# MichaelMillerCSU/Koopman-online-updated-MPC

Hardware: AMD Instinct MI355X
Metric: MPC steps/s (lift+EDMD-update+QP, N=20, 20-dim lift) (higher is better)
Workload: dtype f64

## Files before the change

include/koopmpc.h:

```cpp
#ifndef KOOPMPC_H
#define KOOPMPC_H

#include <stdint.h>

#ifdef __cplusplus
extern "C" {
#endif

typedef struct kmpc_handle kmpc_handle;

enum { KMPC_F32 = 0, KMPC_F64 = 1 };
enum {
  KMPC_LIFT_MLP = 0,
  KMPC_LIFT_RBF_PY = 1,
  KMPC_LIFT_RBF_MATLAB = 2,
  KMPC_LIFT_RBF_GAUSS = 3,
  KMPC_LIFT_RBF_INVQUAD = 4,
  KMPC_LIFT_RBF_INVMULTQUAD = 5,
  KMPC_LIFT_RBF_POLYHARMONIC = 6
};
enum {
  KMPC_OUT_CX = 0,
  KMPC_OUT_LIFT = 1
};
// ... 36 lines not shown
const char* kmpc_last_error(const kmpc_handle* h);
int kmpc_version(void);

int kmpc_set_encoder(kmpc_handle* h, int layer, const double* W_host, const double* b_host,
                     int rows, int cols);
int kmpc_set_encoder_layer(kmpc_handle* h, int layer, const double* W_host, const double* b_host,
                           int rows, int cols);
int kmpc_set_centres(kmpc_handle* h, const double* cx_host, int L, int n);
int kmpc_set_rbf_order(kmpc_handle* h, int k);
int kmpc_set_model(kmpc_handle* h, const double* A_host, const double* B_host, const double* C_host);

int kmpc_set_terminal_weight(kmpc_handle* h, const double* PN);
int kmpc_reset(kmpc_handle* h, void* stream);
int kmpc_state_init(kmpc_handle* h, double P0_scale, double barQ0_scale, void* stream);
int kmpc_state_init_from(kmpc_handle* h, const double* K_A0, const double* P0, const double* barX0,
                         const double* barQ0, void* stream);

int kmpc_lift(kmpc_handle* h, const void* X_dev, void* Psi_dev, int B, void* stream);

int kmpc_rls_update(kmpc_handle* h, const void* psi_dev, const void* u_dev, const void* psi_next_dev,
                    const void* x_next_dev, int B, void* stream);

int kmpc_get_model(kmpc_handle* h, void* A_dev, void* B_dev, void* C_dev, void* stream);

int kmpc_condense(kmpc_handle* h, const void* psi_dev, const void* ref_dev, int ref_per_traj,
                  void* H_dev, void* f_dev, int B, void* stream);
int kmpc_condense_cost(kmpc_handle* h, const void* psi_dev, const void* ref_dev, int ref_per_traj,
                       void* H_dev, void* f_dev, void* c_dev, int B, void* stream);

int kmpc_mpc_solve(kmpc_handle* h, const void* A_dev, const void* B_dev, const void* C_dev, int model_shared,
                   const void* psi_dev, const void* ref_dev, int ref_per_traj, double lb, double ub, double Qw,
                   double Rw, const double* PN_host, void* U_dev, void* U0_dev, void* fun_dev, int32_t* status_dev,
                   int32_t* iters_dev, int B, void* stream);

int kmpc_qp_solve(kmpc_handle* h, const void* H_dev, const void* f_dev, void* U_dev,
                  int32_t* status_dev, int32_t* iters_dev, int B, void* stream);

int kmpc_step(kmpc_handle* h, const void* X_dev, const void* ref_dev, int ref_per_traj,
              void* U0_dev, void* Useq_dev, int32_t* status_dev, int32_t* iters_dev, void* stream);

int64_t kmpc_gram_elems(const kmpc_handle* h);
int kmpc_allreduce_gram(kmpc_handle* h, double* delta_gram_dev, void* nccl_comm, void* stream);
int kmpc_shared_local_gram(kmpc_handle* h, const void* X_dev, double* delta_gram_dev, void* stream);
int kmpc_gram_accumulate(kmpc_handle* h, const void* X_dev, double* delta_gram_dev, void* stream);
int kmpc_shared_solve(kmpc_handle* h, const double* delta_gram_dev, const void* ref_dev, void* U0_dev,
                      void* Useq_dev, int32_t* status_dev, int32_t* iters_dev, void* stream);
int kmpc_shared_solve_plant(kmpc_handle* h, const double* delta_gram_dev, const void* ref_dev, void* U0_dev, void* Useq_dev,
                            int32_t* status_dev, int32_t* iters_dev, int plant, void* X_dev, int switched, double hstep,
                            void* stream);
int kmpc_shared_rollout(kmpc_handle* h, int plant, void* X_dev, const void* ref_dev, int steps, int step0, int switch_step, double hstep,
                        void* nccl_comm, void* U_log_dev, void* X_log_dev, void* U0_dev, void* Useq_dev, int32_t* status_dev,
                        int32_t* iters_dev, void* stream);
int kmpc_shared_get_model(kmpc_handle* h, void* A_dev, void* B_dev, void* C_dev, void* stream);

int kmpc_offline_fit(kmpc_handle* h, const void* X_dev, const void* Y_dev, const void* U_dev, int M,
                     double ridge, int init_rls, void* A_dev, void* B_dev, void* C_dev, void* stream);
int kmpc_generate_and_fit(kmpc_handle* h, int plant, const void* X0_dev, const void* U_dev, int n_traj, int n_steps,
                          double hstep, double ridge, int init_rls, void* A_dev, void* B_dev, void* C_dev,
                          void* X_out_dev, void* Y_out_dev, void* stream);

int kmpc_set_applied_input(kmpc_handle* h, const void* U_dev, int B, void* stream);

int kmpc_plant_step(kmpc_handle* h, int plant, void* X_dev, const void* U_dev, double hstep,
                    int switched, int B, void* stream);

int kmpc_rollout(kmpc_handle* h, int plant, void* X_dev, const void* ref_dev, int ref_per_traj,
                 int steps, int step0, int switch_step, double hstep, void* U_log_dev, void* X_log_dev,
                 int32_t* status_dev, int32_t* iters_dev, void* stream);

int kmpc_solve_dare(const void* A, const void* B, const double* Q, double R, int maxiter, double eps, int nb,
                    int L, void* P, void* K, int32_t* iters, void* stream);
int kmpc_terminal_from_dare(kmpc_handle* h, const double* Q, double R, int maxiter, double eps,
                            int per_trajectory, double* PN_out, int32_t* iters_out, void* stream);

int kmpc_set_terminal_refresh(kmpc_handle* h, int every, const double* Q_host, double R, int maxiter, double eps);

int64_t kmpc_state_bytes(const kmpc_handle* h);
int kmpc_state_export(kmpc_handle* h, void* host_blob, int64_t bytes);
int kmpc_state_import(kmpc_handle* h, const void* host_blob, int64_t bytes);

int kmpc_profile_enable(kmpc_handle* h, int on);
int kmpc_profile_read(kmpc_handle* h, double* ms2, int64_t* count, int reset);
int kmpc_rollout_is_fused(const kmpc_handle* h);
int kmpc_rollout_plugin_status(const kmpc_handle* h, char* text, int text_bytes);
int kmpc_rollout_plugin_prebuild(int n, int L, int N, int out_rows, int lift_kind, int hidden_eff, int batch, int dtype, char* text,
                                 int text_bytes);
int kmpc_rank_by_work(const int32_t* work_dev, int B, int32_t* perm_dev, void* stream);
int kmpc_set_rollout_workgroup(int trajectories);
int64_t kmpc_algorithmic_bytes_per_step(const kmpc_handle* h);
int kmpc_set_online_update(kmpc_handle* h, int on);

int kmpc_set_rollout_diagnostics(kmpc_handle* h, int on);
int kmpc_rollout_diag(kmpc_handle* h, int plant, void* X_dev, const void* ref_dev, int ref_per_traj, int steps, int step0,
                      int switch_step, double hstep, void* U_log_dev, void* X_log_dev, void* Psi_log_dev, void* dA_log_dev,
                      void* dB_log_dev, void* dC_log_dev, int32_t* status_dev, int32_t* iters_dev, void* stream);
int kmpc_estimator_status(const kmpc_handle* h, double* P0, double* barQ0);
int kmpc_get_prev_transition(kmpc_handle* h, void* psi_prev_dev, void* u_prev_dev, void* stream);
int kmpc_rollout_diag_plugin_prebuild(int n, int L, int N, int out_rows, int lift_kind, int hidden_eff, int batch, int with_term,
                                      char* text, int text_bytes);

#ifdef __cplusplus
}
#endif
#endif
```

koopman-online-updated-mpc_amd/csrc/api.hip:

```cpp
#include <hip/hip_runtime.h>

#include <cmath>
#include <cstdio>
#include <cstring>
#include <string>
#include <vector>

#include "../../include/koopmpc.h"
#include "kernels.h"
#include <dlfcn.h>
#include <rccl/rccl.h>

using namespace kmpc;

static thread_local std::string g_create_error;

struct kmpc_handle {
  kmpc_config cfg{};
  std::string err;
  virtual ~kmpc_handle() {
    for (auto& mk : marks) (void)hipEventDestroy(mk.e);
  }
  virtual int set_encoder_layer(int layer, const double* W, const double* b, int rows, int cols) = 0;
  virtual int set_centres(const double* cx, int L, int n) = 0;
  virtual int set_rbf_order(int k) = 0;
  virtual int set_model(const double* A, const double* B, const double* C) = 0;
  virtual int set_terminal_weight(const double* PN) = 0;
  virtual int terminal_from_dare(const double* Qh, double R, int maxiter, double eps, int per_traj, double* PN_out,
                                 int32_t* iters_out, hipStream_t s) = 0;
  virtual int set_terminal_refresh(int every, const double* Qh, double R, int maxiter, double eps) = 0;
  virtual int rollout_is_fused() const = 0;
  virtual int rollout_plugin_status(std::string* text) const = 0;
  virtual int reset(hipStream_t s) = 0;
  virtual int state_init(double P0, double barQ0, hipStream_t s) = 0;
  virtual int state_init_from(const double* KA0, const double* P0m, const double* barX0, const double* barQ0m, hipStream_t s) = 0;
  virtual int lift(const void* X, void* Psi, int B, hipStream_t s) = 0;
  virtual int rls_update(const void* psi, const void* u, const void* psin, const void* xn, int B, hipStream_t s) = 0;
  virtual int get_model(void* A, void* B, void* C, hipStream_t s) = 0;
  virtual int condense(const void* psi, const void* ref, int rpt, void* H, void* f, void* c, int B, hipStream_t s) = 0;
  virtual int mpc_solve(const void* A, const void* Bv, const void* C, int shared, const void* psi, const void* ref, int rpt,
                        double lb, double ub, double Qw, double Rw, const double* PN, void* U, void* U0, void* fun,
                        int32_t* st, int32_t* it, int B, hipStream_t s) = 0;
  virtual int generate_and_fit(int plant, const void* X0, const void* U, int n_traj, int n_steps, double hs, double ridge,
                               int init_rls, void* A, void* B, void* C, void* Xo, void* Yo, hipStream_t s) = 0;
  int device = 0;
  struct StreamMark { hipStream_t s; hipEvent_t e; unsigned long long age; };
  std::vector<StreamMark> marks;
  unsigned long long mark_clock = 0;
  void mark_stream(hipStream_t s) {
    hipStreamCaptureStatus cap = hipStreamCaptureStatusNone;
    if (hipStreamIsCapturing(s, &cap) != hipSuccess) { (void)hipGetLastError(); return; }
    if (cap != hipStreamCaptureStatusNone) return;
    StreamMark* m = nullptr;
    for (auto& mk : marks)
      if (mk.s == s) { m = &mk; break; }
    if (!m) {
      if (marks.size() >= 16) {
        m = &marks[0];
        for (auto& mk : marks)
          if (mk.age < m->age) m = &mk;
        (void)hipEventSynchronize(m->e);
        m->s = s;
      } else {
        hipEvent_t e = nullptr;
        if (hipEventCreateWithFlags(&e, hipEventDisableTiming) != hipSuccess) { (void)hipGetLastError(); return; }
        marks.push_back(StreamMark{s, e, 0});
        m = &marks.back();
      }
    }
    m->age = ++mark_clock;
    if (hipEventRecord(m->e, s) != hipSuccess) (void)hipGetLastError();
  }
  hipError_t sync_marks() {
    for (auto& mk : marks) {
      const hipError_t e = hipEventSynchronize(mk.e);
      if (e != hipSuccess) return e;
    }
    return hipSuccess;
  }
  virtual int qp_solve(const void* H, const void* f, void* U, int32_t* st, int32_t* it, int B, hipStream_t s) = 0;
  virtual int step(const void* X, const void* ref, int rpt, void* U0, void* Useq, int32_t* st, int32_t* it,
                   hipStream_t s) = 0;
  virtual int plant_step(int plant, void* X, const void* U, double h, int sw, int B, hipStream_t s) = 0;
  virtual int set_applied_input(const void* U, int B, hipStream_t s) = 0;
  virtual int set_online_update(int on) = 0;
  virtual int rollout(int plant, void* X, const void* ref, int rpt, int steps, int step0, int switch_step, double hs,
                      void* Ulog, void* Xlog, int32_t* st, int32_t* it, hipStream_t s) = 0;
  virtual int set_rollout_diagnostics(int on) = 0;
  virtual int estimator_status(double* P0, double* barQ0) const = 0;
  virtual int get_prev_transition(void* psi_prev, void* u_prev, hipStream_t s) = 0;
  virtual int rollout_diag(int plant, void* X, const void* ref, int rpt, int steps, int step0, int switch_step, double hs, void* Ulog,
                           void* Xlog, void* Psilog, void* dAlog, void* dBlog, void* dClog, int32_t* st, int32_t* it, hipStream_t s) = 0;
  virtual int offline_fit(const void* X, const void* Y, const void* U, int M, double ridge, int init_rls, void* A,
                          void* B, void* C, hipStream_t s) = 0;
  virtual int64_t gram_elems() const = 0;
  virtual int shared_local_gram(const void* X, double* delta, hipStream_t s) = 0;
  virtual int shared_solve_plant(const double* delta, const void* ref, void* U0, void* Useq, int32_t* st, int32_t* it, int plant, void* X,
                                 int switched, double hstep, hipStream_t s) = 0;
  virtual int shared_solve(const double* delta, const void* ref, void* U0, void* Useq, int32_t* st, int32_t* it,
                           hipStream_t s) = 0;
  virtual int shared_get_model(void* A, void* B, void* C, hipStream_t s) = 0;
  virtual int shared_rollout(int plant, void* X, const void* ref, int steps, int step0, int switch_step, double hstep, void* comm,
                             void* Ulog, void* Xlog, void* U0out, void* Useq, int32_t* st, int32_t* it, hipStream_t s) = 0;
  virtual int64_t state_bytes() const = 0;
  virtual int state_export(void* blob, int64_t bytes) = 0;
  virtual int state_import(const void* blob, int64_t bytes) = 0;
  virtual int profile_enable(int on) = 0;
  virtual int profile_read(double* ms2, int64_t* count, int reset) = 0;
  virtual int64_t algorithmic_bytes() const = 0;
};

static void* resolve_nccl_allreduce() {
  static void* fn = nullptr;
  if (!fn) {
// ... 997 lines not shown
      if ((rc = pack_encoder(s))) return rc;
      r.lift_rbf = 0;
      r.W1 = dW1; r.b1 = db1; r.Whp[0] = dWhp[0]; r.Whp[1] = dWhp[1]; r.bh[0] = dbh[0]; r.bh[1] = dbh[1];
      r.Wop = dWop; r.bo = dbo; r.Hp = enc.Hp; r.Lp = enc.Lp; r.KS = enc.KS; r.nhh = cfg.layers - 1;
    } else {
      r.lift_rbf = 1;
      r.cx = dcx; r.eps = (T)cfg.rbf_eps; r.rbf_matlab = rbf_code();
    }
    r.psi[0] = dPsi[0]; r.psi[1] = dPsi[1]; r.cur = cur;
    r.steps = steps; r.step0 = step0; r.switch_step = switch_step;
    r.have_prev = have_prev ? 1 : 0; r.rls_fresh = rls_fresh ? 1 : 0;
    r.no_update = update_on ? 0 : 1;
    r.U_log = (T*)Ulog; r.X_log = (T*)Xlog;
    r.io_f32 = io32 ? 1 : 0;
    if (io32 && !r.s.U0) r.s.U0 = dU0;
    if (ctx.diag) { r.diag = 1; r.Psi_log = (T*)ctx.diag->Psi; r.dA_log = (T*)ctx.diag->dA; r.dB_log = (T*)ctx.diag->dB; r.dC_log = (T*)ctx.diag->dC; }
    if constexpr (sizeof(T) == 8) {
      if (term_every > 0) {
        if (io32) FAIL(-3, "the per-step terminal refresh is a float64 feature");
        r.term_every = term_every; r.term_count0 = (int)(term_count % term_every); r.term_maxiter = term_maxiter;
        r.term_R = term_R; r.term_eps = term_eps; r.term_Q = dTermQ; r.term_W = dWtB;
        r.term_scratch = dTermScr; r.term_scratch_stride = term_scratch_elems(L); r.term_iters = dDareIt;
        r.s.Wterm = dWtB; r.s.wterm_per_traj = 1;
      }
    }
    const bool global_place = cfg.lift_kind == KMPC_LIFT_MLP && (B & 15) == 0 && B <= (1 << 20);
    if (!dbg_env("KMPC_ROLLOUT_NO_PLACE")) {
      if (!dWork) {
        HIPCHK(hipMalloc(&dWork, sizeof(int32_t) * (size_t)B));
        HIPCHK(hipMemsetAsync(dWork, 0, sizeof(int32_t) * (size_t)B, s));
      }
      r.work = dWork;
      static const int tail = dbg_env("KMPC_PLACE_TAIL") ? atoi(dbg_env("KMPC_PLACE_TAIL")) : 5;
      r.work_tail = tail;
      if (place_valid && global_place && !dbg_env("KMPC_ROLLOUT_NO_GLOBAL_PLACE")) r.perm = dPerm;
      if (evPlace && place_stream != s) HIPCHK(hipStreamWaitEvent(s, evPlace, 0));
    }
    if constexpr (sizeof(T) == 8) {
      if (use_img) {
        if ((rc = ensure_image(s))) return rc;
        r.img = dImg; r.img_stride = sImg;
      } else if ((rc = ensure_dense(s, true))) return rc;
    }
    bool rec;
    if ((rc = prof_begin(s, &rec)) || (rec && (rc = prof_mid(s)))) return rc;
    HIPCHK(launch_rollout_fused<T>(r, s, &variant_of(ctx.diag != nullptr).plugin));
    if (rec && (rc = prof_end(s, steps))) return rc;
    if (r.work && steps >= 4 && global_place) {
      if (!dPerm) HIPCHK(hipMalloc(&dPerm, sizeof(int32_t) * (size_t)B * 3));
      HIPCHK(launch_place(dWork, B, dPerm, reinterpret_cast<uint32_t*>(dPerm + B), s));
      place_valid = true;
    } else {
      place_valid = false;
    }
    if (r.work) {
      if (!evPlace) HIPCHK(hipEventCreateWithFlags(&evPlace, hipEventDisableTiming));
      HIPCHK(hipEventRecord(evPlace, s));
      place_stream = s;
    }
    if (term_every > 0) term_count += steps;
    if (update_on && (steps >= 2 || (steps == 1 && have_prev))) rls_fresh = false;
    have_prev = true;
    cur ^= (steps & 1);
    return 0;
  }

  T* dU0 = nullptr;
  int rollout(int plant, void* X, const void* ref, int rpt, int steps, int step0, int switch_step, double hs,
              void* Ulog, void* Xlog, int32_t* st, int32_t* it, hipStream_t s) override {
    return rollout_impl(StepCtx{}, plant, X, ref, rpt, steps, step0, switch_step, hs, Ulog, Xlog, st, it, s);
  }
  int rollout_impl(const StepCtx& ctx, int plant, void* X, const void* ref, int rpt, int steps, int step0, int switch_step, double hs,
                   void* Ulog, void* Xlog, int32_t* st, int32_t* it, hipStream_t s) {
    if (!X || !ref || steps < 0) FAIL(-3, "kmpc_rollout: bad arguments");
    if (!dU0) HIPCHK(hipMalloc(&dU0, sizeof(T) * (size_t)B));
    if (n != 2) FAIL(-3, "plants are two-state systems");
    if (!plant_id_ok(plant)) FAIL(-3, "unknown plant");
    const bool fused = fused_rollout_ok() && (!ctx.diag || diag_fused_ready());
    const bool kernel_writes_totals = steps > 0 && fused && cfg.lift_kind == KMPC_LIFT_MLP;
    if (!kernel_writes_totals) {
      if (st) HIPCHK(hipMemsetAsync(st, 0, sizeof(int32_t) * (size_t)B, s));
      if (it) HIPCHK(hipMemsetAsync(it, 0, sizeof(int32_t) * (size_t)B, s));
    }
    if (steps > 0 && fused)
      return rollout_fused(ctx, plant, X, ref, rpt, steps, step0, switch_step, hs, Ulog, Xlog, st, it, s);
    if (steps == 0 && fused) {
      if constexpr (sizeof(T) == 8) {
        if (use_img) return ensure_image(s);
      } else if (core) {
        int rc = ensure_image(s);
        if (!rc && core->use_img && (rc = core->ensure_image(s))) err = core->err;
        return rc;
      }
      return 0;
    }
    for (int i = 0; i < steps; ++i) {
      const int gi = step0 + i;
      T* u = Ulog ? (T*)Ulog + (size_t)i * B : dU0;
      if (ctx.diag) { const int rcd = diag_before_step(*ctx.diag, X, i, s); if (rcd) return rcd; }
      int rc = step_impl(StepCtx{true, plant, (switch_step >= 0 && gi >= switch_step) ? 1 : 0, hs, X, nullptr}, X, ref, rpt, u, nullptr, st, it, s);
      if (rc) return rc;
      if (Xlog) HIPCHK(hipMemcpyAsync((T*)Xlog + (size_t)i * n * B, X, sizeof(T) * (size_t)n * B,
                                      hipMemcpyDeviceToDevice, s));
    }
    return 0;
  }

  double *dGram = nullptr, *dPartial = nullptr;
  T *dKs = nullptr, *dCs = nullptr, *dHs = nullptr, *dFs = nullptr, *df0s = nullptr, *dTs = nullptr;
  double* dFastPack = nullptr;
  bool fast_pack_valid = false;
  int32_t* dNeed = nullptr;
  int32_t* dWork = nullptr;
  int32_t* dPerm = nullptr;
  bool place_valid = false;
  hipEvent_t evPlace = nullptr;
  hipStream_t place_stream = nullptr;
  int32_t* dQpList = nullptr;
  int qp_list_parity = 0;
  T* dWt = nullptr;
  std::vector<double> hostPN;
  bool have_wterm = false;
  double* dDareP = nullptr; int32_t* dDareIt = nullptr; double* dWtB = nullptr;
  int dare_cap = 0;
  bool wterm_from_dare = false, wterm_per_traj = false;
  bool shared_has_samples = false;
  static constexpr int GRAM_BLOCKS = 256;
  int64_t gram_elems() const override { return (int64_t)(p + L + n) * p; }
  int shared_alloc() {
    if (dGram) return 0;
    const int R = p + L + n, MT = (R + 15) / 16, NT = (p + 15) / 16;
    HIPCHK(hipMalloc(&dGram, sizeof(double) * (size_t)R * p));
    HIPCHK(hipMemset(dGram, 0, sizeof(double) * (size_t)R * p));
    HIPCHK(hipMalloc(&dPartial, sizeof(double) * (size_t)GRAM_BLOCKS * MT * 16 * NT * 16));
    HIPCHK(hipMalloc(&dKs, sizeof(T) * (size_t)L * p));
    HIPCHK(hipMalloc(&dCs, sizeof(T) * (size_t)n * L));
    HIPCHK(hipMalloc(&dHs, sizeof(T) * (size_t)N * N));
    HIPCHK(hipMalloc(&dFs, sizeof(T) * (size_t)N * (L + 1)));
    HIPCHK(hipMalloc(&df0s, sizeof(T) * (size_t)N));
    { int rc = sync_own(); if (rc) return rc; }
    { int rc = ensure_dense(nullptr, false); if (rc) return rc; HIPCHK(hipStreamSynchronize(nullptr)); }
    HIPCHK(hipMemcpy(dKs, dK, sizeof(T) * (size_t)L * p, hipMemcpyDeviceToDevice));
    HIPCHK(hipMemcpy(dCs, dC, sizeof(T) * (size_t)n * L, hipMemcpyDeviceToDevice));
    return 0;
  }
  int shared_local_gram(const void* X, double* delta, hipStream_t s) override {
    if (!X || !delta) FAIL(-3, "kmpc_shared_local_gram: null pointer");
    int rc = shared_alloc();
    if (rc) return rc;
    if (core && (rc = ensure_dense(s, true))) return rc;
    T* psi_now = dPsi[cur];
    T* psi_prev = dPsi[cur ^ 1];
    GramArgs<T> g{};
    g.B = B; g.n = n; g.L = L; g.max_blocks = GRAM_BLOCKS;
    g.psi_prev = psi_prev; g.pp_sl = 1; g.pp_sb = L;
    g.psi_now = psi_now; g.pn_sl = 1; g.pn_sb = L;
    g.u_prev = dUprev; g.x_now = (const T*)X; g.partial = dPartial;
    if constexpr (sizeof(T) == 8) {
      const bool two = dbg_env("KMPC_SHARED_LIFT_GRAM_2") != nullptr;
      if (have_prev && !two && cfg.lift_kind == KMPC_LIFT_MLP) {
        if ((rc = check_lift_ready())) return rc;
        LiftArgs<T> a{};
        a.B = B; a.n = n; a.L = L; a.hidden = enc.hid; a.nlayers = cfg.layers;
        a.X = (const T*)X; a.Psi = psi_now; a.ps_l = 1; a.ps_b = L;
        a.W1 = dW1; a.b1 = db1; a.Wh[0] = dWh[0]; a.Wh[1] = dWh[1]; a.bh[0] = dbh[0]; a.bh[1] = dbh[1];
        a.Wo = dWo; a.bo = dbo; a.Hp = enc.Hp; a.Lp = enc.Lp;
        if ((rc = pack_encoder(s))) return rc;
        a.Whp[0] = dWhp[0]; a.Whp[1] = dWhp[1] ? dWhp[1] : dWhp[0]; a.Wop = dWop; a.KSp = enc.KS;
// ... 351 lines not shown
    return 0;
  }

  int64_t algorithmic_bytes() const override {
    const int64_t s = sizeof(T);
    return s * (2 * ((int64_t)p * p + L * p + L * L + n * L) + (L + L * p + n * L + N * m + n) + (n + m + q * N));
  }
};

struct DeviceGuard {
  int prev = -1;
  explicit DeviceGuard(int dev) { if (hipGetDevice(&prev) != hipSuccess) prev = -1; if (prev != dev) (void)hipSetDevice(dev); else prev = -1; }
  ~DeviceGuard() { if (prev >= 0) (void)hipSetDevice(prev); }
};
extern "C" {

int kmpc_version(void) { return 100; }

int kmpc_create(const kmpc_config* cfg, kmpc_handle** out) {
  if (!cfg || !out) { g_create_error = "kmpc_create: null argument"; return -1; }
  *out = nullptr;
  int ndev = 0;
  if (hipGetDeviceCount(&ndev) != hipSuccess || ndev == 0) {
    g_create_error = "kmpc_create: no HIP device visible (libkoopmpc has no CPU path)";
    return -5;
  }
  kmpc_handle* h = nullptr;
  int rc;
  if (cfg->dtype == KMPC_F64) { auto* i = new Impl<double>(); rc = i->init(*cfg); h = i; }
  else if (cfg->dtype == KMPC_F32) { auto* i = new Impl<float>(); rc = i->init(*cfg); h = i; }
  else { g_create_error = "kmpc_create: dtype must be KMPC_F32 or KMPC_F64"; return -2; }
  if (rc) { g_create_error = h->err; delete h; return rc; }
  if (hipGetDevice(&h->device) != hipSuccess) h->device = 0;
  *out = h;
  return 0;
}

int kmpc_destroy(kmpc_handle* h) {
  if (!h) return 0;
  DeviceGuard g(h->device);
  delete h;
  return 0;
}
const char* kmpc_last_error(const kmpc_handle* h) { return h ? h->err.c_str() : g_create_error.c_str(); }

#define NN(h) if (!(h)) return -1; DeviceGuard dev_guard_((h)->device)
struct StreamMarkAtExit {
  kmpc_handle* h; hipStream_t s;
  ~StreamMarkAtExit() { h->mark_stream(s); }
};
#define NNS(h, s) NN(h); StreamMarkAtExit mark_at_exit_{(h), (hipStream_t)(s)}
int kmpc_set_encoder(kmpc_handle* h, int layer, const double* W, const double* b, int rows, int cols) { NN(h); return h->set_encoder_layer(layer, W, b, rows, cols); }
int kmpc_set_encoder_layer(kmpc_handle* h, int layer, const double* W, const double* b, int rows, int cols) { return kmpc_set_encoder(h, layer, W, b, rows, cols); }
int kmpc_set_centres(kmpc_handle* h, const double* cx, int L, int n) { NN(h); return h->set_centres(cx, L, n); }
int kmpc_set_rbf_order(kmpc_handle* h, int k) { NN(h); return h->set_rbf_order(k); }
int kmpc_set_model(kmpc_handle* h, const double* A, const double* B, const double* C) { NN(h); return h->set_model(A, B, C); }
int kmpc_set_terminal_weight(kmpc_handle* h, const double* PN) { NN(h); return h->set_terminal_weight(PN); }
int kmpc_terminal_from_dare(kmpc_handle* h, const double* Q, double R, int maxiter, double eps, int per_trajectory,
                            double* PN_out, int32_t* iters_out, void* s) {
  NNS(h, s);
  return h->terminal_from_dare(Q, R, maxiter, eps, per_trajectory, PN_out, iters_out, (hipStream_t)s);
}
int kmpc_solve_dare(const void* A, const void* B, const double* Q, double R, int maxiter, double eps, int nb, int L,
                    void* P, void* K, int32_t* iters, void* s) {
  if (nb == 0) return 0;
  if (!A || !B || !Q || !P || nb < 0 || L < 1 || L > 64 || maxiter < 1) return -3;
  double* dQl = nullptr;
  if (hipMalloc(&dQl, sizeof(double) * (size_t)L * L) != hipSuccess) return -1001;
  int rc = 0;
  if (hipMemcpyAsync(dQl, Q, sizeof(double) * (size_t)L * L, hipMemcpyHostToDevice, (hipStream_t)s) != hipSuccess) rc = -1002;
  DareArgs d{};
  d.nb = nb; d.L = L; d.q = 0; d.maxiter = maxiter; d.shared_model = 0;
  d.A = (const double*)A; d.strideA = (long)L * L; d.ldA = L;
  d.B = (const double*)B; d.strideB = L; d.incB = 1;
  d.Q = dQl; d.R = R; d.eps = eps; d.Co = nullptr; d.strideC = 0;
  d.P = (double*)P; d.K = (double*)K; d.PN = nullptr; d.pn_sub_diag = 0.0; d.iters = iters;
  if (!rc && launch_dare(d, (hipStream_t)s) != hipSuccess) rc = -1003;
  if (hipStreamSynchronize((hipStream_t)s) != hipSuccess && !rc) rc = -1004;
  (void)hipFree(dQl);
  return rc;
}
int kmpc_set_terminal_refresh(kmpc_handle* h, int every, const double* Q, double R, int maxiter, double eps) { NN(h); return h->set_terminal_refresh(every, Q, R, maxiter, eps); }
int kmpc_rollout_is_fused(const kmpc_handle* h) { NN(h); return h->rollout_is_fused(); }
static void put_text(char* text, int text_bytes, const std::string& t) { if (text && text_bytes > 0) snprintf(text, (size_t)text_bytes, "%s", t.c_str()); }
static int prebuild_variant(int n, int L, int N, int q, bool rbf, int hidden_eff, int batch, bool io32, bool term, bool diag, std::string* text, bool rbf_kinds) {
  const EncoderShape e = encoder_shape(hidden_eff, 0, n, L);
  RolloutPluginKey k{};
  if (!rollout_plugin_key(n, L, N, q, rbf, e.Lp, e.KS, e.Hp, batch, io32, &k, term, diag, rbf_kinds)) return 0;
  if (!rollout_plugin_get(k, text)) return -1;
  *text = rollout_plugin_describe(k);
  return 1;
}
int kmpc_rollout_plugin_prebuild(int n, int L, int N, int out_rows, int lift_kind, int hidden_eff, int batch, int dtype, char* text, int text_bytes) {
  auto say = [&](int code, const std::string& t) { put_text(text, text_bytes, t); return code; };
  const bool rbf = lift_kind != KMPC_LIFT_MLP, io32 = dtype == KMPC_F32;
  const int q = out_rows > 0 ? out_rows : n;
  if (lift_kind < KMPC_LIFT_MLP || lift_kind > KMPC_LIFT_RBF_POLYHARMONIC) return say(-3, "lift_kind must be one of KMPC_LIFT_* (0..6)");
  if (n != 2 || L < 1 || N < 1 || batch < 1 || (!rbf && (hidden_eff < 1 || hidden_eff > 128)) || (dtype != KMPC_F32 && dtype != KMPC_F64)) return say(-3, "bad arguments");
  if (!(io32 ? rollout_io32_available(n, L, N, q, rbf) : rollout_fused_available<double>(n, L, N, q, 64, rbf))) return say(2, "no fused roll-out for this configuration");
  std::string t;
  const int rc = prebuild_variant(n, L, N, q, rbf, hidden_eff, batch, io32, false, false, &t, lift_kind >= KMPC_LIFT_RBF_GAUSS);
  return rc == 0 ? say(0, "built-in instantiation of libkoopmpc.so") : say(rc, t);
}
int kmpc_rollout_diag_plugin_prebuild(int n, int L, int N, int out_rows, int lift_kind, int hidden_eff, int batch, int with_term, char* text, int text_bytes) {
  auto say = [&](int code, const std::string& t) { put_text(text, text_bytes, t); return code; };
  const bool rbf = lift_kind != KMPC_LIFT_MLP;
  const int q = out_rows > 0 ? out_rows : n;
  if (lift_kind < KMPC_LIFT_MLP || lift_kind > KMPC_LIFT_RBF_POLYHARMONIC) return say(-3, "lift_kind must be one of KMPC_LIFT_* (0..6)");
  if (n != 2 || L < 1 || N < 1 || batch < 1 || (!rbf && (hidden_eff < 1 || hidden_eff > 128))) return say(-3, "bad arguments");
  std::string t;
  const int rc = rollout_fused_available<double>(n, L, N, q, 64, rbf) ? prebuild_variant(n, L, N, q, rbf, hidden_eff, batch, false, with_term != 0, true, &t, lift_kind >= KMPC_LIFT_RBF_GAUSS) : 0;
  return rc == 0 ? say(2, "no fused diagnostics variant for this configuration (per-step launches)") : say(rc, t);
}
int kmpc_rollout_plugin_status(const kmpc_handle* h, char* text, int text_bytes) {
  if (!h) return -100;
  std::string t;
  const int rc = h->rollout_plugin_status(&t);
  put_text(text, text_bytes, t);
  return rc;
}
int kmpc_rank_by_work(const int32_t* work_dev, int B, int32_t* perm_dev, void* s) {
  if (!work_dev || !perm_dev) return -3;
  const hipError_t e = kmpc::launch_place(work_dev, B, perm_dev, reinterpret_cast<uint32_t*>(perm_dev + B), (hipStream_t)s);
  return e == hipSuccess ? 0 : -(1000 + (int)e);
}
int kmpc_set_rollout_workgroup(int trajectories) {
  if (trajectories != 0 && trajectories != 4 && trajectories != 8 && trajectories != 16) return -1;
  kmpc::set_rollout_workgroup(trajectories);
  return 0;
}
int kmpc_reset(kmpc_handle* h, void* s) { NNS(h, s); return h->reset((hipStream_t)s); }
int kmpc_state_init(kmpc_handle* h, double P0_scale, double barQ0_scale, void* s) { NNS(h, s); return h->state_init(P0_scale, barQ0_scale, (hipStream_t)s); }
int kmpc_state_init_from(kmpc_handle* h, const double* K_A0, const double* P0, const double* barX0, const double* barQ0, void* s) {
  NNS(h, s);
  return h->state_init_from(K_A0, P0, barX0, barQ0, (hipStream_t)s);
}
int kmpc_lift(kmpc_handle* h, const void* X, void* Psi, int B, void* s) { NNS(h, s); return h->lift(X, Psi, B, (hipStream_t)s); }
int kmpc_rls_update(kmpc_handle* h, const void* psi, const void* u, const void* psin, const void* xn, int B, void* s) { NNS(h, s); return h->rls_update(psi, u, psin, xn, B, (hipStream_t)s); }
int kmpc_get_model(kmpc_handle* h, void* A, void* B, void* C, void* s) { NNS(h, s); return h->get_model(A, B, C, (hipStream_t)s); }
int kmpc_condense(kmpc_handle* h, const void* psi, const void* ref, int rpt, void* H, void* f, int B, void* s) { NNS(h, s); return h->condense(psi, ref, rpt, H, f, nullptr, B, (hipStream_t)s); }
int kmpc_condense_cost(kmpc_handle* h, const void* psi, const void* ref, int rpt, void* H, void* f, void* c, int B, void* s) { NNS(h, s); return h->condense(psi, ref, rpt, H, f, c, B, (hipStream_t)s); }
int kmpc_mpc_solve(kmpc_handle* h, const void* A, const void* Bv, const void* C, int shared, const void* psi, const void* ref, int rpt,
                   double lb, double ub, double Qw, double Rw, const double* PN, void* U, void* U0, void* fun, int32_t* st, int32_t* it,
                   int B, void* s) {
  NNS(h, s);
  return h->mpc_solve(A, Bv, C, shared, psi, ref, rpt, lb, ub, Qw, Rw, PN, U, U0, fun, st, it, B, (hipStream_t)s);
}
int kmpc_generate_and_fit(kmpc_handle* h, int plant, const void* X0, const void* U, int n_traj, int n_steps, double hs, double ridge,
                          int init_rls, void* A, void* B, void* C, void* Xo, void* Yo, void* s) {
  NNS(h, s);
  return h->generate_and_fit(plant, X0, U, n_traj, n_steps, hs, ridge, init_rls, A, B, C, Xo, Yo, (hipStream_t)s);
}
int kmpc_qp_solve(kmpc_handle* h, const void* H, const void* f, void* U, int32_t* st, int32_t* it, int B, void* s) { NNS(h, s); return h->qp_solve(H, f, U, st, it, B, (hipStream_t)s); }
int kmpc_step(kmpc_handle* h, const void* X, const void* ref, int rpt, void* U0, void* Useq, int32_t* st, int32_t* it, void* s) { NNS(h, s); return h->step(X, ref, rpt, U0, Useq, st, it, (hipStream_t)s); }
int kmpc_set_applied_input(kmpc_handle* h, const void* U, int B, void* s) { NNS(h, s); return h->set_applied_input(U, B, (hipStream_t)s); }
int kmpc_set_online_update(kmpc_handle* h, int on) { NN(h); return h->set_online_update(on); }
int kmpc_plant_step(kmpc_handle* h, int plant, void* X, const void* U, double hs, int sw, int B, void* s) { NNS(h, s); return h->plant_step(plant, X, U, hs, sw, B, (hipStream_t)s); }
int kmpc_rollout(kmpc_handle* h, int plant, void* X, const void* ref, int rpt, int steps, int step0, int sw, double hs, void* Ulog, void* Xlog, int32_t* st, int32_t* it, void* s) { NNS(h, s); return h->rollout(plant, X, ref, rpt, steps, step0, sw, hs, Ulog, Xlog, st, it, (hipStream_t)s); }
int kmpc_set_rollout_diagnostics(kmpc_handle* h, int on) { NN(h); return h->set_rollout_diagnostics(on); }
int kmpc_estimator_status(const kmpc_handle* h, double* P0, double* barQ0) { if (!h) return -1; return h->estimator_status(P0, barQ0); }
int kmpc_get_prev_transition(kmpc_handle* h, void* psi_prev, void* u_prev, void* s) { NNS(h, s); return h->get_prev_transition(psi_prev, u_prev, (hipStream_t)s); }
int kmpc_rollout_diag(kmpc_handle* h, int plant, void* X, const void* ref, int rpt, int steps, int step0, int sw, double hs, void* Ulog, void* Xlog,
                      void* Psilog, void* dAlog, void* dBlog, void* dClog, int32_t* st, int32_t* it, void* s) {
  NNS(h, s);
  return h->rollout_diag(plant, X, ref, rpt, steps, step0, sw, hs, Ulog, Xlog, Psilog, dAlog, dBlog, dClog, st, it, (hipStream_t)s);
}
// ... 34 lines not shown
```

koopman-online-updated-mpc_amd/csrc/kernels.h:

```cpp
#pragma once
#include <hip/hip_runtime.h>
#include <stdint.h>

#include <string>

namespace kmpc {

const char* dbg_env(const char* name);


enum { PH_RLS = 1, PH_CONDENSE = 2, PH_QP = 4 };
enum { OUT_CX = 0, OUT_LIFT = 1 };

template <typename T>
struct StepArgs {
  int B, n, L, q, N;
  int out_kind;
  int phases;
  int first_update;
  int max_iter;
  int ref_per_traj;
  int accumulate;
  int du_mode;
  int cy0;
// ... 40 lines not shown
  T* Psi; long ps_l, ps_b;
  const T* W1; const T* b1;
  const T* Wh[2]; const T* bh[2];
  const T* Wo; const T* bo;
  int Hp, Lp;
  const T* Whp[2]; const T* Wop; int KSp;
  const T* cx; T eps; int rbf_matlab;
};

template <typename T> struct RolloutArgs {
  StepArgs<T> s;
  int lift_rbf;
  const T* W1; const T* b1;
  const T* Whp[2]; const T* bh[2];
  const T* Wop; const T* bo;
  int Hp, Lp, KS, nhh;
  const T* cx; T eps; int rbf_matlab;
  T* psi[2];
  int cur;
  int steps, step0, switch_step, have_prev, rls_fresh;
  int no_update;
  int wstride;
  int wbase;
  int keep_off;
  T* U_log; T* X_log;
  T* img; long img_stride;
  int io_f32;
  int32_t* work;
  int work_tail;
  const int32_t* perm;
  int term_every, term_count0, term_maxiter;
  T term_R, term_eps;
  const T* term_Q;
  T* term_W;
  T* term_scratch;
  long term_scratch_stride;
  int32_t* term_iters;
  int diag;
  T* Psi_log; T* dA_log; T* dB_log; T* dC_log;
};
static constexpr long term_scratch_elems(int L) { return 4L * L * L + 5L * L + 16; }
hipError_t launch_place(const int32_t* work, int B, int32_t* perm, uint32_t* scratch, hipStream_t s);

template <typename T> struct GramArgs {
  int B, n, L, max_blocks;
  const T* psi_prev; long pp_sl, pp_sb;
  const T* psi_now;  long pn_sl, pn_sb;
  const T* u_prev; const T* x_now;
  double* partial;
};

template <typename T> struct PlantArgs {
  int B, plant, switched; T h; T* X; const T* U;
};

struct DareArgs {
  int nb, L, q, maxiter, shared_model;
  const double* A; long strideA; int ldA;
  const double* B; long strideB; int incB;
  const double* Q;
  double R, eps;
  const double* Co; long strideC;
  double* P;
  double* K;
  double* PN;
  double pn_sub_diag;
  int32_t* iters;
};
hipError_t launch_dare(const DareArgs& a, hipStream_t s);

size_t step_lds_bytes(int n, int L, int q, int N, size_t elem, int* r1, int* r2, bool lds_tableau = true);

#define KMPC_PLUGIN_ABI 6003
template <typename T> hipError_t launch_step(const StepArgs<T>& a, int threads, hipStream_t s);
template <typename T> bool rollout_fused_available(int n, int L, int N, int q, int threads, bool rbf);
void set_rollout_workgroup(int trajectories);
struct RolloutPluginKey { int L, N, q, nw, ks, io32, term, diag; };
typedef hipError_t (*rollout_plugin_fn)(const RolloutArgs<double>* a, int waves, hipStream_t s);
bool rollout_plugin_dims(int n, int L, int N, int q);
rollout_plugin_fn rollout_plugin_get(const RolloutPluginKey& k, std::string* err);
std::string rollout_plugin_describe(const RolloutPluginKey& k);
struct RolloutPlugin { RolloutPluginKey key{}; rollout_plugin_fn fn = nullptr; };
template <typename T> hipError_t launch_rollout_fused(const RolloutArgs<T>& a, hipStream_t s, const RolloutPlugin* plugin);
bool rollout_builtin(int L, int N, int q, bool io32);
bool rollout_plugin_key(int n, int L, int N, int q, bool rbf, int Lp, int KS, int Hp, int B, bool io32, RolloutPluginKey* out, bool term = false,
                        bool diag = false, bool rbf_kinds = false);
struct EncoderShape { int hid, Hp, Lp, KS; };
inline EncoderShape encoder_shape(int hidden, int lift_offset, int n, int L) {
  const int hid = hidden + (lift_offset == 2 ? 2 * n : 0);
  return {hid, hid <= 112 ? 112 : 128, ((L + 15) / 16) * 16, (hid + 3) / 4};
}
struct V2Dims {
  int L, n, p, cp, s2, s1;
  __host__ __device__ V2Dims(int L_, int n_) : L(L_), n(n_), p(L_ + 1), cp((L_ + 2) / 2), s2(2 * L_ + 1), s1(L_ + n_) {}
  __host__ __device__ long elems() const { return (long)cp * (s2 + s1) * 2; }
  __host__ __device__ long off2(int slot, int col) const { return ((long)(col >> 1) * s2 + slot) * 2 + (col & 1); }
  __host__ __device__ long off1(int slot, int col) const { return (long)cp * s2 * 2 + ((long)(col >> 1) * s1 + slot) * 2 + (col & 1); }
};
bool rollout_uses_image(int n, int L, int N, int q);
bool rollout_io32_available(int n, int L, int N, int q, bool rbf);
long state_image_elems(int L, int n);
hipError_t launch_state_to_image(const double* P, long sP, const double* K, long sK, const double* Q, long sQ, const double* C, long sC,
                                 int n, int L, int B, double* img, long stride, hipStream_t s);
hipError_t launch_image_to_state(const double* img, long stride, int n, int L, int B, double* P, long sP, double* K, long sK,
                                 double* Q, long sQ, double* C, long sC, hipStream_t s);
struct RlsDiagArgs {
  int B, n, L;
  int has_update, first_update, use_C;
  const double* P; long strideP; const double* K; long strideK; const double* Qb; long strideQ; const double* C; long strideC;
  const double* psi_prev; const double* psi_now;
  const double* u_prev;
  const double* x_now;
  double* Psi_row;
  double* dA_row; double* dB_row; double* dC_row;
};
hipError_t launch_rls_diag(const RlsDiagArgs& a, hipStream_t s);
template <typename T> hipError_t launch_pack_afrag(const T* src, int Mp, int Hp, int KS, T* dst, hipStream_t s);
bool lift_gram_available(const LiftArgs<double>& a);
hipError_t launch_lift_gram(const LiftArgs<double>& a, const GramArgs<double>& g, int* nblocks, hipStream_t s);
hipError_t launch_gram_reduce(const double* partial, int nblocks, int L, int n, double forget, double* gram, hipStream_t s);
template <typename T> hipError_t launch_lift_mlp(const LiftArgs<T>& a, hipStream_t s);
template <typename T> hipError_t launch_lift_rbf(const LiftArgs<T>& a, hipStream_t s);
template <typename T> hipError_t launch_plant(const PlantArgs<T>& a, hipStream_t s);
template <typename T> hipError_t launch_fill_state(T* P, long strideP, int p, T P0, T* Qb, long strideQ, int L,
                                                   T Q0, T* K, long strideK, T* C, long strideC, int n, int B,
                                                   hipStream_t s);
hipError_t launch_axpby(double* g, const double* d, double a, int count, hipStream_t s);
template <typename S, typename D> hipError_t launch_cast(const S* src, D* dst, size_t count, hipStream_t s);
template <typename T> hipError_t launch_gram(const GramArgs<T>& a, double forget, double* gram, hipStream_t s);
template <typename T> hipError_t launch_shared_solve(const double* gram, int L, int n, double dP, double dQ, int use_C,
                                                     T* Kout, T* Cout, hipStream_t s, T* Pout = nullptr,
                                                     T* Qout = nullptr);
template <typename T> hipError_t launch_shared_condense(const T* K, const T* C, const T* ref, int L, int n, int q, int N,
                                                        int out_kind, double Qw, double Rw, T* Hout, T* Fout, T* f0out,
                                                        hipStream_t s, const T* Wterm = nullptr, int du_mode = 0,
                                                        int cy0 = 0);
template <typename T>
hipError_t launch_shared_model(double* gram, const double* delta, double forget, const T* ref, int Lm, int n, int q, int N, double dP, double dQ, int use_C,
                               int have_samples, double Qw, double Rw, T* Kio, T* Cio, T* Hout, T* Fout, T* f0out, T* Tout,
                               const T* Wt, int du_mode, int cy0, hipStream_t s);
template <typename T>
hipError_t launch_shared_fast(const StepArgs<T>& a, int32_t* need, hipStream_t s);
bool shared_model_available(int Lm, int n, int q, int N, int du_mode);
struct SharedModel2Args {
  double* gram; const double* delta; double forget; const double* ref;
  int Lm, n, q, N;
  double dP, dQ; int have_samples; double Qw, Rw;
  double *Kio, *Cio, *Hout, *Fout, *f0out, *Tout;
  const double* Wt; int du_mode, cy0;
  double* pack; int pack_mt, pack_ks1, pack_ks2;
};
bool shared_fast_shape(int N, int Lf, int* MT, int* KS1, int* KS2);
inline size_t shared_fast_pack_elems(int MT, int KS1, int KS2) { return (size_t)(KS1 + 2 * KS2) * MT * 64; }
bool shared_model2_available(int Lm, int n, int q, int N, int du_mode);
hipError_t launch_shared_model2(const SharedModel2Args& a, hipStream_t s);
template <typename T> hipError_t launch_broadcast(T* dst, long stride, const T* src, int count, int B, hipStream_t s);
template <typename T> hipError_t launch_import_model(const T* A, const T* Bv, const T* C, int shared, int n, int L, int B,
                                                    T* K, long strideK, T* Cs, long strideC, hipStream_t s);
template <typename T> hipError_t launch_datagen(int plant, T h, const T* X0, const T* U, int n_traj, int n_steps, T* X, T* Y,
                                                hipStream_t s);
template <typename T> hipError_t launch_qp_value(const T* H, const T* f, const T* c, const T* U, int N, int B, T* fun, hipStream_t s);
inline int device_slot() { int d = 0; if (hipGetDevice(&d) != hipSuccess || d < 0) d = 0; return d & 15; }
template <typename T> hipError_t launch_export_model(const T* K, long strideK, const T* C, long strideC, int n, int L,
                                                     int B, T* A_out, T* B_out, T* C_out, hipStream_t s);

}
// ... 1 lines not shown
```

koopman-online-updated-mpc_amd/csrc/qp_rl.h:

```cpp
#pragma once
#include "step_body.h"

namespace kmpc {

__device__ __forceinline__ double half_sum(double s) {
  s += dpp_shr(s, 1);
  s += dpp_shr(s, 2);
  s += dpp_shr(s, 4);
  s += dpp_shr(s, 8);
  double rt = 0.0;
  fmac_rowbcast<15, true>(rt, s, 1.0);
  double r0, r1;
  half_gather(rt, r0, r1);
  return r0 + r1;
}
__device__ __forceinline__ void half_sums_u(double s, double& lo, double& hi) {
  s += dpp_shr(s, 1);
  s += dpp_shr(s, 2);
  s += dpp_shr(s, 4);
  s += dpp_shr(s, 8);
  lo = lane_bcast(s, 15) + lane_bcast(s, 31);
  hi = lane_bcast(s, 47) + lane_bcast(s, 63);
}
__device__ __forceinline__ double dpp_shr_keep(double v, int ctrl) {
  const int lo = __double2loint(v), hi = __double2hiint(v);
  switch (ctrl) {
    case 1: return __hiloint2double(__builtin_amdgcn_update_dpp(hi, hi, 0x111, 0xf, 0xf, false), __builtin_amdgcn_update_dpp(lo, lo, 0x111, 0xf, 0xf, false));
    case 2: return __hiloint2double(__builtin_amdgcn_update_dpp(hi, hi, 0x112, 0xf, 0xf, false), __builtin_amdgcn_update_dpp(lo, lo, 0x112, 0xf, 0xf, false));
    case 4: return __hiloint2double(__builtin_amdgcn_update_dpp(hi, hi, 0x114, 0xf, 0xf, false), __builtin_amdgcn_update_dpp(lo, lo, 0x114, 0xf, 0xf, false));
    default: return __hiloint2double(__builtin_amdgcn_update_dpp(hi, hi, 0x118, 0xf, 0xf, false), __builtin_amdgcn_update_dpp(lo, lo, 0x118, 0xf, 0xf, false));
  }
}
__device__ __forceinline__ double half_max(double s) {
  double w;
  w = dpp_shr_keep(s, 1); s = w > s ? w : s;
  w = dpp_shr_keep(s, 2); s = w > s ? w : s;
  w = dpp_shr_keep(s, 4); s = w > s ? w : s;
  w = dpp_shr_keep(s, 8); s = w > s ? w : s;
  double rt = 0.0;
  fmac_rowbcast<15, true>(rt, s, 1.0);
  double r0, r1;
  half_gather(rt, r0, r1);
  return r0 > r1 ? r0 : r1;
}
__device__ __forceinline__ void halves_both_q(double a, double& lo, double& hi) {
  const int al = __double2loint(a), ah = __double2hiint(a);
  const auto rl = __builtin_amdgcn_permlane32_swap(al, al, false, false);
  const auto rh = __builtin_amdgcn_permlane32_swap(ah, ah, false, false);
  lo = __hiloint2double(rh[0], rl[0]);
  hi = __hiloint2double(rh[1], rl[1]);
}
template <int N_> __device__ __forceinline__ void rl_upd(double (&M)[N_], double v0, double v1, double coef) {
  row_upd<N_, -1>(M, v0, v1, coef);
}
template <int N_> __device__ __forceinline__ double rl_matvec(const double (&M)[N_], double v) {
  double v0, v1;
  half_gather(v, v0, v1);
  double ac = 0.0;
  row_dot<N_, (N_ > 16)>(ac, v0, v1, M);
  return ac;
}

template <int N_, int K>
__device__ __forceinline__ void rl_sweep(double (&M)[N_], double& rs, double& rsi, bool rev, double d, int t, int half) {
  asm volatile("" : "+v"(half));
  asm volatile("" : "+v"(t));
  const double dinv = fast_rcp(d);
  const double colk = M[K];
  double v0, v1;
  half_gather(rs * colk, v0, v1);
  const bool isk = t == K;
  const double c = (half || isk) ? 0.0 : -colk * dinv;
  rl_upd<N_>(M, v0, v1, c);
  const double sg = rev ? -1.0 : 1.0;
  if (!half) {
    M[K] = isk ? -sg * rsi : sg * colk * dinv;
    if (isk) { rs *= sg * dinv; rsi *= sg * d; }
  }
}
template <int N_, int K = 0>
__device__ __forceinline__ void rl_sweep_set(double (&M)[N_], double& rs, double& rsi, unsigned diff, unsigned& Smask, unsigned& Fmask,
                                             bool& broke, bool drop, int t, int half) {
  if constexpr (K < N_) {
    if ((diff >> K) & 1u) {
      const bool rev = (Smask >> K) & 1u;
      const double d = lane_bcast(rs * M[K], K);
      if (!((rev ? -d : d) > 0.0)) {
        broke = true;
        if (drop) Fmask &= ~(1u << K);
      } else {
        rl_sweep<N_, K>(M, rs, rsi, rev, d, t, half);
        Smask ^= (1u << K);
      }
    }
    rl_sweep_set<N_, K + 1>(M, rs, rsi, diff, Smask, Fmask, broke, drop, t, half);
  }
}

constexpr int rl_stride(int N) { return ((((N + 1) & ~1) / 2) & 1) ? ((N + 1) & ~1) : ((N + 1) & ~1) + 2; }

struct QpCarry {
  unsigned smask;
  int valid;
  unsigned umask;
  int trust;
};

template <int N_, typename IOT = double>
__device__ __forceinline__ bool qp_rl(double* const sR, const double* sf, const StepArgs<double>& a, const StepVar<double>& sv, const int b,
                                      double* qx_out, double* u_slot, double (&M)[N_], double& rs, double& rsi, QpCarry& cs, double up, double xw_pre) {
  typedef double d2_t __attribute__((ext_vector_type(2)));
  static_assert(N_ <= 32, "qp_rl: one variable per lane of a 32-lane half (ownmask, row_newbcast index, diagonal lane)");
  const int tid = local_tid<64>(), half = tid >> 5, t = tid & 31;
  const bool own = t < N_;
  const int B = a.B;
  const double uprev = a.du_mode ? up : 0.0;
  double lb = a.lb, ub = a.ub;
  const double tol = Tol<double>::kkt();
  const double eact = Tol<double>::act() * (ub - lb);
  const double xmaxb = tabs(lb) > tabs(ub) ? tabs(lb) : tabs(ub);
  if (a.du_mode && t == 0) {
    lb = (a.umin - uprev) > lb ? (a.umin - uprev) : lb;
    ub = (a.umax - uprev) < ub ? (a.umax - uprev) : ub;
  }
  const double c0 = tclip(0.0, lb, ub);
  const bool warm = a.x_warm != nullptr, predict_on = (a.qp_predict & 1) != 0;
  const int max_iter = a.max_iter;
  constexpr unsigned ownmask = N_ >= 32 ? 0xffffffffu : ((1u << N_) - 1u);
  const int rowi = own ? t : N_ - 1;
  constexpr int NS = rl_stride(N_);
  const double* const hrow = sR + rowi * NS;
  auto load_h_rows = [&]() {
    if constexpr ((N_ & 1) == 0) {
      const d2_t* h2 = reinterpret_cast<const d2_t*>(__builtin_assume_aligned(hrow, 16));
#pragma unroll
      for (int j = 0; j < N_ / 2; ++j) { const d2_t v = h2[j]; M[2 * j] = v.x; M[2 * j + 1] = v.y; }
    } else {
#pragma unroll
      for (int j = 0; j < N_; ++j) M[j] = hrow[j];
    }
  };
  bool carried = cs.valid != 0;
  const int nstale0 = cs.trust & 0xff, probe_age = (cs.trust >> 8) & 0xff;
  const bool full_budget = nstale0 < 2 || probe_age >= 3;
  const int kr_max = full_budget ? 8 : 3;
  bool went_stale = false;
  const bool carried_at_start = carried;
  unsigned Smask = carried ? cs.smask : 0u;
  if (half || !carried) load_h_rows();
  if (!carried) {
    if (!half) {
#pragma unroll
      for (int j = 0; j < N_; ++j) M[j] *= 2.0;
    }
    rs = 1.0; rsi = 1.0;
  }
  const double fi = own ? sf[t] : 0.0;
  double ra = 0.0;
#pragma unroll
  for (int j = 0; j < N_; ++j) ra += tabs(M[j]);
  {
    double lo, hi;
    halves_both_q(ra, lo, hi);
    ra = hi;
  }
  const double gs = tabs(fi) + 2.0 * ra * xmaxb;
  const bool held = carried && !warm && !((Smask >> t) & 1u);
  double x = own ? (warm ? tclip(xw_pre, lb, ub) : (held ? (((cs.umask >> t) & 1u) ? ub : lb) : c0)) : 0.0;
  double hx;
  {
    double lo, hi;
    halves_both_q(rl_matvec<N_>(M, x), lo, hi);
    hx = own ? hi : 0.0;
  }
  double J0 = 0.0, Jhi;
  bool Jok = false;
  int it = 0, status = 1, refresh = 0, polish = 0, rtot = 0, ncrawl = 0, nref = 0;
  bool nopredict = false, rebuild = false;
#ifdef KMPC_TRACE
  int tc_sweeps = 0, tc_rebuild = 0, tc_pass = 0, tc_ls = 0, tc_mv = 1;
  const bool tc_carried0 = carried;
#define KCOUNT(x) (x)
#else
#define KCOUNT(x)
#endif
  KTRACE(8);

  while (true) {
    double g = 0.0;
    bool bad = false, inI = false, loose = false;
    if (own) {
      g = 2.0 * hx + fi;
      const bool atl = x <= lb + eact, atu = x >= ub - eact;
      inI = (atl && (g > 0.0)) || (atu && (g < 0.0));
      const double viol = inI ? 0.0 : tabs(g);
      const double res = tabs(x - tclip(x - g, lb, ub));
      const double xs = tabs(x) > 1.0 ? tabs(x) : 1.0;
      bad = !((viol <= tol * gs) || (res <= tol * xs));
      loose = viol > Tol<double>::tight() * gs;
    }
    const unsigned Bmask = (unsigned)__ballot(bad);
    const bool refine = (unsigned)__ballot(loose) != 0u;
    const unsigned Imask = (unsigned)__ballot(inI);
    if ((unsigned)__ballot(own && !(tabs(g) <= 1e300)) != 0u || (Jok && (!(J0 == J0) || tabs(J0) > 1e300))) { status = 2; break; }
    if (Bmask == 0u && (it > 0 || !warm)) {
      if (!refine || polish >= 2) { status = 0; break; }
      ++polish;
    }
    if (it >= max_iter || refresh > 4) { status = 1; break; }
    if (it >= N_ || ncrawl >= N_ + 4) { status = 3; break; }
// ... 79 lines not shown
      if (own) g += 2.0 * sR[t * NS + jl] * delta;
      Fmask &= ~(1u << jl);
      ++rounds;
    }
    if (it == 0) KTRACE(11);

    double alpha = 1.0, xa = x, hxa = 0.0, Ja = J0;
    bool redo = false;
    while (true) {
      double dstep = pdir;
      if (!isF) {
        const double g0 = 2.0 * hx + fi;
        dstep = own ? ((g0 > 0.0 ? lb : (g0 < 0.0 ? ub : x)) - x) : 0.0;
        if (rounds > 0 && own && !inI) dstep = qx_out[t] - x;
      }
      const double xu = x + alpha * dstep;
      xa = own ? tclip(xu, lb, ub) : 0.0;
      const bool plain = alpha == 1.0 && rounds == 0 && (unsigned)__ballot(own && (isF ? xa != xu : xa != x)) == 0u;
      if (plain) {
        hxa = own ? hx + hp : 0.0;
      } else {
        double lo, hi;
        halves_both_q(rl_matvec<N_>(M, xa), lo, hi);
        hxa = own ? hi : 0.0;
      }
      if (plain && exact) {
        Jok = false;
        break;
      }
      if (!Jok) {
        half_sums_u(own ? x * (hx + fi) : 0.0, J0, Jhi);
        Jok = true;
      }
      const double pJa = own ? xa * (hxa + fi) : 0.0;
      if (rounds > 0) {
        half_sums_u(pJa, Ja, Jhi);
        if (!(Ja <= J0)) redo = true;
        break;
      }
      const double pdec = own ? (isF ? alpha * (-g * pdir) : g * (x - xa)) : 0.0;
      double sD;
      half_sums_u(half ? pdec : pJa, Ja, sD);
      const double mag = tabs(J0) > tabs(Ja) ? tabs(J0) : tabs(Ja);
      if ((J0 - Ja >= 1e-4 * sD - Tol<double>::slack() * mag) || alpha < 1e-10) break;
      if (carried) { redo = true; break; }
      alpha *= 0.25;
      KCOUNT(++tc_ls);
      ++ncrawl;
    }
    if (redo) {
      if (carried && rounds == 0) { rebuild = true; continue; }
      nopredict = true;
      ncrawl += 3;
      continue;
    }
    nopredict = false;
    rtot += rounds;
    x = xa;
    hx = hxa;
    if (Jok) J0 = Ja;
    if (it == 0) KTRACE(12);
    ++it;
  }
  KTRACE(13);
#ifdef KMPC_TRACE
  if (tid == 0 && b < 8192) {
    kmpc_trace_buf[b * 32 + 15] = (unsigned long long)(it + rtot);
    kmpc_trace_buf[b * 32 + 22] += (unsigned long long)tc_sweeps;
    kmpc_trace_buf[b * 32 + 23] += (unsigned long long)tc_rebuild;
    kmpc_trace_buf[b * 32 + 24] += (unsigned long long)tc_pass;
    kmpc_trace_buf[b * 32 + 25] += (unsigned long long)it;
    kmpc_trace_buf[b * 32 + 26] += (unsigned long long)(tc_ls + rtot * 1000);
    kmpc_trace_buf[b * 32 + 27] += (unsigned long long)((tc_carried0 ? 1 : 0) + ((it == 1 && tc_sweeps == 0 && tc_rebuild == 0 && rtot == 0) ? 1000 : 0));
    (void)tc_mv;
  }
#endif
  if (status == 2) x = own ? c0 : 0.0;
  if (status == 3) {
    if (own && !half) qx_out[t] = x;
    cs.valid = 0;
    return true;
  }
  if (own && !half) {
    if (a.Useq) io_st<IOT>(a.Useq, (size_t)t * B + b, x);
    if (a.x_warm) a.x_warm[(size_t)t * B + b] = x;
  }
  if (tid == 0) {
    const double uout = a.du_mode ? uprev + x : x;
    *u_slot = x;
    if (sv.U0) io_st<IOT>(sv.U0, b, uout);
    if (a.u_store) a.u_store[b] = uout;
    if (a.plant >= 0) {
      double x1, x2;
      if (sv.x_next) { x1 = lds_ld(sv.x_next); x2 = lds_ld(sv.x_next + 1); }
      else { x1 = io_ld<IOT>(a.X_rw, b); x2 = io_ld<IOT>(a.X_rw, (size_t)B + b); }
      plant_apply<double>(a.plant, sv.plant_switched, a.plant_h, x1, x2, uout);
      io_st<IOT>(a.X_rw, b, x1);
      io_st<IOT>(a.X_rw, (size_t)B + b, x2);
      if (sv.x_next) { lds_st(sv.x_next, x1); lds_st(sv.x_next + 1, x2); }
    }
    if (sv.x_next) {
      lds_i32* const acc = (lds_i32*)reinterpret_cast<int*>(sv.x_next + 2);
      acc[0] = acc[0] > status ? acc[0] : status;
      acc[1] += it + rtot;
      acc[2] += 8 * (it + rtot - 1) + 5 * nref + (carried ? 3 * __builtin_popcount(cs.smask ^ Smask) : 3 * N_);
    } else {
      if (a.status) a.status[b] = a.accumulate ? (a.status[b] > status ? a.status[b] : status) : status;
      if (a.iters) a.iters[b] = a.accumulate ? a.iters[b] + it + rtot : it + rtot;
    }
  }
  const bool keep = status == 0 && !(carried && (it >= 4 || nref >= 7));
  if (keep && own && !half) {
    double* const trow = sR + t * NS;
    if constexpr ((N_ & 1) == 0) {
      d2_t* t2 = reinterpret_cast<d2_t*>(__builtin_assume_aligned(trow, 16));
#pragma unroll
      for (int j = 0; j < N_ / 2; ++j) { d2_t v; v.x = M[2 * j]; v.y = M[2 * j + 1]; t2[j] = v; }
    } else {
#pragma unroll
      for (int j = 0; j < N_; ++j) trow[j] = M[j];
    }
  }
  cs.valid = keep ? 1 : 0;
  if (carried_at_start) {
    const int ns = went_stale ? (nstale0 < 255 ? nstale0 + 1 : 255) : 0;
    const int age = full_budget ? 0 : probe_age + 1;
    cs.trust = ns | (age << 8);
  }
  cs.smask = Smask;
  cs.umask = (unsigned)__ballot(own && x >= ub - eact);
  KTRACE(14);
  return false;
}

}
```

koopman-online-updated-mpc_amd/csrc/rollout_kernel.hip:

```cpp
#include "step_body.h"
#include "step_v2.h"
#include "dare_device.h"
#ifdef KMPC_ROLLOUT_JIT_TU
#define dbg_env(name) ((const char*)nullptr)
#endif

namespace kmpc {

typedef double d4_t __attribute__((ext_vector_type(4)));
#ifdef KMPC_TRACE
#define LSTAMP(i)                                                                                      \
  do {                                                                                                 \
    if (wv == 0 && lane == 0 && b0 < 8192) kmpc_lift_buf[(b0 >> 4) * 16 + (i)] = wall_clock64();      \
  } while (0)
__device__ unsigned long long kmpc_lift_buf[512 * 16];
extern "C" int kmpc_lift_trace_read(void* host, size_t bytes) {
  return (int)hipMemcpyFromSymbol(host, HIP_SYMBOL(kmpc_lift_buf), bytes, 0, hipMemcpyDeviceToHost);
}
__device__ unsigned kmpc_step_buf[4096 * 96];
extern "C" int kmpc_step_trace_read(void* host, size_t bytes) {
  return (int)hipMemcpyFromSymbol(host, HIP_SYMBOL(kmpc_step_buf), bytes, 0, hipMemcpyDeviceToHost);
}
#else
#define LSTAMP(i)
// ... 46 lines not shown
  typedef double d4_t __attribute__((ext_vector_type(4)));
  typedef const double __attribute__((address_space(1))) * gp_t;
  typedef double __attribute__((address_space(3))) * lp_t;
  auto uni = [](int v) { return __builtin_amdgcn_readfirstlane(v); };
  auto unip = [&](const double* q) {
    const unsigned long long a = (unsigned long long)q;
    const unsigned lo = (unsigned)__builtin_amdgcn_readfirstlane((int)(unsigned)a), hi = (unsigned)__builtin_amdgcn_readfirstlane((int)(unsigned)(a >> 32));
    return (gp_t)(((unsigned long long)hi << 32) | lo);
  };
  const int wv = uni(wv_), KSr = uni(KSr_), nhh = uni(nhh_), b0 = uni(b0_);
  (void)b0;
  const bool hid = uni(hid_ ? 1 : 0) != 0, out = uni(out_ ? 1 : 0) != 0;
  const gp_t W1 = unip(W1_), b1 = unip(b1_), Wh0 = unip(Wh0_), Wh1 = unip(Wh1_), Wo = unip(Wo_), bh0 = unip(bh0_), bh1 = unip(bh1_), bo = unip(bo_);
  const lp_t sXn = (lp_t)sXn_, sAct0 = (lp_t)sAct0_, sAct1 = (lp_t)sAct1_, sPsi = (lp_t)sPsi_;
  constexpr int AR = NW == 8 ? 32 : 64;
  const int bl = NW == 8 ? ((lane >> 4) << 3) + (lane & 7) : lane;
  const int KS = KS_ > 0 ? KS_ : KSr;
  double af[2][RO_KB2];
  auto loadf = [&](gp_t Wp_, int ks0, double (&dst)[RO_KB2]) {
#pragma unroll
    for (int i = 0; i < RO_KB2; ++i) dst[i] = ks0 + i < KS ? Wp_[((size_t)wv * KS + ks0 + i) * 64 + lane] : 0.0;
  };
  if (nhh > 0) { if (hid) loadf(Wh0, 0, af[0]); }
  else if (out) loadf(Wo, 0, af[0]);
  double a1 = 0.0;
  d4_t c1 = {0.0, 0.0, 0.0, 0.0};
  if (hid) {
    a1 = W1[4 * (16 * wv + (lane & 15)) + (lane >> 4)];
#pragma unroll
    for (int r = 0; r < 4; ++r) c1[r] = b1[16 * wv + (lane >> 4) + 4 * r];
  }
  __syncthreads();
  LSTAMP(0);
  if (hid) {
    c1 = __builtin_amdgcn_mfma_f64_16x16x4f64(a1, sXn[4 * (lane & 15) + (lane >> 4)], c1, 0, 0, 0);
#pragma unroll
    for (int r = 0; r < 4; ++r) {
      const int row = 16 * wv + (lane >> 4) + 4 * r;
      if (NW != 8 || (lane & 15) < 8) sAct0[(row >> 2) * AR + (row & 3) * (AR / 4) + (lane & 15)] = c1[r] > 0.0 ? c1[r] : 0.0;
    }
  }
  LSTAMP(1);
  __syncthreads();
  LSTAMP(2);
  for (int h = 0; h <= nhh; ++h) {
    const bool last = h == nhh;
    const bool mine = last ? out : hid;
    const lp_t act = (h & 1) ? sAct1 : sAct0;
    const lp_t actn = (h & 1) ? sAct0 : sAct1;
    const gp_t Wp = last ? Wo : ((h & 1) ? Wh1 : Wh0);
    const gp_t bias = last ? bo : ((h & 1) ? bh1 : bh0);
    d4_t acc0 = {0.0, 0.0, 0.0, 0.0}, acc1 = {0.0, 0.0, 0.0, 0.0};
    if (mine) {
#pragma unroll
      for (int r = 0; r < 4; ++r) acc0[r] = bias[16 * wv + (lane >> 4) + 4 * r];
#pragma unroll
      for (int bt = 0; bt < 32 / RO_KB2; ++bt) {
        const int kb = bt * RO_KB2;
        if (kb + RO_KB2 < KS) loadf(Wp, kb + RO_KB2, af[(bt + 1) & 1]);
#pragma unroll
        for (int i = 0; i < RO_KB2; i += 2) {
          if (kb + i < KS) acc0 = __builtin_amdgcn_mfma_f64_16x16x4f64(af[bt & 1][i], act[(kb + i) * AR + bl], acc0, 0, 0, 0);
          if (kb + i + 1 < KS) acc1 = __builtin_amdgcn_mfma_f64_16x16x4f64(af[bt & 1][i + 1], act[(kb + i + 1) * AR + bl], acc1, 0, 0, 0);
        }
      }
      const int col = lane & 15;
#pragma unroll
      for (int r = 0; r < 4; ++r) {
        const int row = 16 * wv + (lane >> 4) + 4 * r;
        const double v = acc0[r] + acc1[r];
        if (last) sPsi[row * 16 + col] = v;
        else if (NW != 8 || col < 8) actn[(row >> 2) * AR + (row & 3) * (AR / 4) + col] = v > 0.0 ? v : 0.0;
      }
    }
    if (!last) {
      if (h + 1 < nhh) { if (hid) loadf(((h + 1) & 1) ? Wh1 : Wh0, 0, af[0]); }
      else if (out) loadf(Wo, 0, af[0]);
    }
    LSTAMP(3 + 2 * h);
    __syncthreads();
    LSTAMP(4 + 2 * h);
  }
}
template <int L_, int N_, int Q_, int NW, int KS_, typename IOT = double, bool TERM = false, bool DIAG = false>
__global__ __launch_bounds__((ro_max_threads<L_, N_, Q_, NW, KS_>())) void rollout_kernel(const RolloutArgs<double> ra) {
  static_assert(sizeof(IOT) == 8 || ro_v2<L_, N_, Q_>(), "float32 I/O: register-state dimension sets only");
  static_assert(!DIAG || (sizeof(IOT) == 8 && ro_v2<L_, N_, Q_>()), "diagnostics: float64 register-state dimension sets only");
  extern __shared__ __attribute__((aligned(16))) unsigned char smem_raw[];
  double* const smem = reinterpret_cast<double*>(smem_raw);
  constexpr int NC = NW == 4 ? 4 : 16;
  constexpr bool RBF = KS_ < 0;
  const int tid0 = threadIdx.x;
  const int wave = __builtin_amdgcn_readfirstlane(tid0 >> 6);
  const int B = ra.s.B, n = ra.s.n, L = L_;
  const int b0 = blockIdx.x * (int)(blockDim.x >> 6);
  double* const sAct0 = smem;
  double* const sAct1 = sAct0 + (NW == 8 ? ro_act8() : RO_ACT);
  double* const sPsi = smem + ra.keep_off;
  double* const sXn = sPsi + ra.Lp * NC;
  int slot_traj = wave;
  if constexpr (!RBF && NW == 16) {
    if (ra.perm) {
      slot_traj = b0 + wave < B ? ra.perm[b0 + wave] - b0 : wave;
    } else if (ra.work) {
      int* const sHint = reinterpret_cast<int*>(sPsi);
      int* const sRank = sHint + 16;
      if (tid0 < 16) sHint[tid0] = b0 + (int)tid0 < B ? ra.work[b0 + tid0] : -1;
      __syncthreads();
      if (tid0 < 16) {
        const int ht = sHint[tid0];
        int r = 0;
        for (int v = 0; v < 16; ++v) { const int hv = sHint[v]; r += (hv > ht || (hv == ht && v < (int)tid0)) ? 1 : 0; }
        sRank[r] = tid0;
      }
      __syncthreads();
      slot_traj = __builtin_amdgcn_readfirstlane(sRank[wave]);
      __syncthreads();
    }
  }
  const int b = b0 + slot_traj;
  const bool live = b < B;
  if (!RBF && tid0 < 4 * NC) sXn[tid0] = 0.0;
  __syncthreads();
  if (!RBF && (tid0 & 63) < 4)
    sXn[wave * 4 + (tid0 & 63)] = (live && (int)(tid0 & 63) < n) ? io_ld<IOT>(ra.s.X_rw, (size_t)(tid0 & 63) * B + b) : 0.0;

  if constexpr (ro_v2<L_, N_, Q_>()) {
    if (live) step_v2_init<L_, N_, Q_>(smem + ra.wbase + wave * ra.wstride);
  }
  bool have_prev = ra.have_prev != 0, fresh = ra.rls_fresh != 0;
  int cur = ra.cur;
  constexpr bool V2 = ro_v2<L_, N_, Q_>();
  constexpr int PSI_MASK = V2 ? 31 : 63;
  double psi_prev_reg = 0.0;
  if (live && ra.have_prev && (int)(tid0 & PSI_MASK) < L) psi_prev_reg = ra.psi[ra.cur ^ 1][(size_t)b * L + (tid0 & PSI_MASK)];
  typedef const RolloutArgs<double> __attribute__((address_space(4))) * kernarg_ptr_t;
  for (int k = 0; k < ra.steps; ++k) {
    kernarg_ptr_t kp = (kernarg_ptr_t)__builtin_amdgcn_kernarg_segment_ptr();
    asm volatile("" : "+s"(kp));
    const RolloutArgs<double> __attribute__((address_space(4)))& R = *kp;
    const StepArgs<double>& a = *(const StepArgs<double>*)(&kp->s);
    int wv = wave;
    asm volatile("" : "+s"(wv));
    const int lane = local_tid<64>();
    (void)wv;
#ifdef KMPC_TRACE
    if (lane == 0 && b < 8192) kmpc_trace_buf[b * 32 + 16] = wall_clock64();
#endif
    if constexpr (!RBF) {
      if (R.work_tail > 0 && k == R.steps - R.work_tail && lane == 0) ((lds_i32*)reinterpret_cast<int*>(sXn + wv * 4 + 2))[2] = 0;
    }
    double psi_i = 0.0;
    if constexpr (RBF) {
      if (live && (lane & PSI_MASK) < L) {
        const double x0 = io_ld<IOT>(a.X_rw, (size_t)b), x1 = io_ld<IOT>(a.X_rw, (size_t)B + b);
        const double* c = R.cx + (size_t)(lane & PSI_MASK) * n;
        if constexpr (KS_ == -2) psi_i = kmpc_rbf_kind2(x0, x1, c[0], c[1], R.eps, R.rbf_matlab);
        else psi_i = kmpc_rbf_psi2(x0, x1, c[0], c[1], R.eps, R.rbf_matlab);
      }
    } else if constexpr (NW == 4) {
      constexpr int CG = NW / 4;
      constexpr int NT = 8 / NW;
      const int KS = KS_ > 0 ? KS_ : R.KS, Hp = KS_ > 0 ? (KS_ <= 28 ? 112 : 128) : R.Hp, MTH = Hp >> 4, MTO = R.Lp >> 4;
      const int boff = (lane >> 4) * NC + (lane & 3);
      const int drow = ((lane >> 2) & 3) * 4 + (lane >> 4);
      const int dcol = lane & 3;
      const int th0 = wv, th1 = wv + NW;
      const bool vh0 = th0 < MTH, vh1 = NT > 1 && th1 < MTH;
      const int to0 = NW - 1 - wv;
      const bool vo0 = to0 < MTO;
      double af[2][RO_KB2];
      double a1[NT], c1[NT];
#pragma unroll
      for (int t = 0; t < NT; ++t) {
        const int th = wv + t * NW;
        const bool v = th < MTH;
        a1[t] = v ? R.W1[4 * (16 * th + (lane & 15)) + (lane >> 4)] : 0.0;
        c1[t] = v ? R.b1[16 * th + drow] : 0.0;
      }
      if (R.nhh > 0) { if (vh0) ro_load_afrags(R.Whp[0], KS, th0, 0, lane, af[0]); }
      else if (vo0) ro_load_afrags(R.Wop, KS, to0, 0, lane, af[0]);
      __syncthreads();
#pragma unroll
      for (int t = 0; t < NT; ++t) {
        const int th = wv + t * NW;
        if (th < MTH) {
#pragma unroll
          for (int cg = 0; cg < CG; ++cg) {
            const double xb = sXn[(cg * 4 + (lane & 3)) * 4 + (lane >> 4)];
            const double v = __builtin_amdgcn_mfma_f64_4x4x4f64(a1[t], xb, c1[t], 0, 0, 0);
            sAct0[(16 * th + drow) * NC + cg * 4 + dcol] = v > 0.0 ? v : 0.0;
          }
        }
      }
      __syncthreads();
      for (int h = 0; h <= R.nhh; ++h) {
        const bool last = h == R.nhh;
        const int t0 = last ? to0 : th0, t1 = th1;
        const bool v0 = last ? vo0 : vh0, v1 = last ? false : vh1;
        const double* act = (h & 1) ? sAct1 : sAct0;
        double* actn = (h & 1) ? sAct0 : sAct1;
        const double* Wp = last ? R.Wop : R.Whp[h & 1];
        const double* bias = last ? R.bo : R.bh[h & 1];
        double acc[NT][CG][2];
#pragma unroll
        for (int t = 0; t < NT; ++t) {
          const double bv = (t ? v1 : v0) ? bias[16 * (t ? t1 : t0) + drow] : 0.0;
#pragma unroll
          for (int cg = 0; cg < CG; ++cg) { acc[t][cg][0] = bv; acc[t][cg][1] = 0.0; }
        }
        constexpr int NB = 32 / RO_KB2;
#pragma unroll
        for (int g = 0; g < NT * NB; ++g) {
          const int tl = g / NB, kb = (g % NB) * RO_KB2;
          if (g + 1 < NT * NB) {
            const int tl2 = (g + 1) / NB, kb2 = ((g + 1) % NB) * RO_KB2;
            if ((tl2 ? v1 : v0) && kb2 < KS) ro_load_afrags(Wp, KS, tl2 ? t1 : t0, kb2, lane, af[(g + 1) & 1]);
          }
          if ((tl ? v1 : v0) && kb < KS) {
#pragma unroll
            for (int i = 0; i < RO_KB2; ++i)
              if (kb + i < KS) {
#pragma unroll
                for (int cg = 0; cg < CG; ++cg)
                  acc[tl][cg][i & 1] = __builtin_amdgcn_mfma_f64_4x4x4f64(af[g & 1][i], act[(kb + i) * 4 * NC + boff + 4 * cg],
                                                                         acc[tl][cg][i & 1], 0, 0, 0);
              }
          }
        }
#pragma unroll
        for (int t = 0; t < NT; ++t) {
          if (t ? v1 : v0) {
            const int tt = t ? t1 : t0;
#pragma unroll
            for (int cg = 0; cg < CG; ++cg) {
              const double v = acc[t][cg][0] + acc[t][cg][1];
              if (last) sPsi[(16 * tt + drow) * NC + cg * 4 + dcol] = v;
              else actn[(16 * tt + drow) * NC + cg * 4 + dcol] = v > 0.0 ? v : 0.0;
            }
          }
        }
        if (!last) {
          if (h + 1 < R.nhh) { if (vh0) ro_load_afrags(R.Whp[h + 1], KS, th0, 0, lane, af[0]); }
          else if (vo0) ro_load_afrags(R.Wop, KS, to0, 0, lane, af[0]);
        }
        __syncthreads();
      }
      if ((lane & PSI_MASK) < L) psi_i = sPsi[(lane & PSI_MASK) * NC + wv];
    } else {
      const int KS = KS_ > 0 ? KS_ : R.KS, Hp = KS_ > 0 ? (KS_ <= 28 ? 112 : 128) : R.Hp, MTH = Hp >> 4, MTO = R.Lp >> 4;
      const bool hid = wv < MTH, out = wv < MTO;
      if (V2 && !hid && !out) {
        __syncthreads();
        if constexpr (V2) {
          if (live && k > 0 && !R.no_update) {
            int woff0 = R.wbase + wv * R.wstride, bk0 = b;
            asm volatile("" : "+s"(woff0), "+s"(bk0));
            double* const wsm0 = smem + woff0;
            const double uk = a.u_prev[bk0];
            const int t0 = lane & 31;
            const double z0 = t0 < L_ ? psi_prev_reg : (t0 == L_ ? uk : 0.0);
            const double gains0 = v2_rls_cov<L_, true>(R.img + (size_t)bk0 * R.img_stride, z0, a.lam);
            if (lane < 32 || t0 < L_) v2_cov_slot<N_>(wsm0)[v2_cov_index<L_>(lane)] = gains0;
          } else {
            __syncthreads();
            __syncthreads();
          }
        }
        for (int i = 0; i < R.nhh; ++i) __syncthreads();
      } else if constexpr (ro_encoder_call<L_, N_, Q_>()) {
        ro_encoder_tiles<KS_, NW>(wv, lane, b0, KS, hid, out, R.nhh, R.W1, R.b1, R.Whp[0], R.Whp[1], R.Wop, R.bh[0], R.bh[1], R.bo, sXn, sAct0, sAct1, sPsi);
      } else {
      constexpr int AR = NW == 8 ? 32 : 64;
      const int bl = NW == 8 ? ((lane >> 4) << 3) + (lane & 7) : lane;
      double af[2][RO_KB2];
      if (R.nhh > 0) { if (hid) ro_load_afrags(R.Whp[0], KS, wv, 0, lane, af[0]); }
      else if (out) ro_load_afrags(R.Wop, KS, wv, 0, lane, af[0]);
      double a1 = 0.0;
      d4_t c1 = {0.0, 0.0, 0.0, 0.0};
      if (hid) {
        a1 = R.W1[4 * (16 * wv + (lane & 15)) + (lane >> 4)];
#pragma unroll
        for (int r = 0; r < 4; ++r) c1[r] = R.b1[16 * wv + (lane >> 4) + 4 * r];
      }
      __syncthreads();
      LSTAMP(0);
      if (hid) {
        c1 = __builtin_amdgcn_mfma_f64_16x16x4f64(a1, sXn[4 * (lane & 15) + (lane >> 4)], c1, 0, 0, 0);
#pragma unroll
        for (int r = 0; r < 4; ++r) {
          const int row = 16 * wv + (lane >> 4) + 4 * r;
          if (NW != 8 || (lane & 15) < 8) sAct0[(row >> 2) * AR + (row & 3) * (AR / 4) + (lane & 15)] = c1[r] > 0.0 ? c1[r] : 0.0;
        }
      }
      LSTAMP(1);
      __syncthreads();
      LSTAMP(2);
      for (int h = 0; h <= R.nhh; ++h) {
        const bool last = h == R.nhh;
        const bool mine = last ? out : hid;
        const double* act = (h & 1) ? sAct1 : sAct0;
        double* actn = (h & 1) ? sAct0 : sAct1;
        const double* Wp = last ? R.Wop : R.Whp[h & 1];
        const double* bias = last ? R.bo : R.bh[h & 1];
        d4_t acc0 = {0.0, 0.0, 0.0, 0.0}, acc1 = {0.0, 0.0, 0.0, 0.0};
        if (mine) {
#pragma unroll
          for (int r = 0; r < 4; ++r) acc0[r] = bias[16 * wv + (lane >> 4) + 4 * r];
        }
        if (mine) {
#pragma unroll
          for (int bt = 0; bt < 32 / RO_KB2; ++bt) {
            const int kb = bt * RO_KB2;
            if (kb + RO_KB2 < KS) ro_load_afrags(Wp, KS, wv, kb + RO_KB2, lane, af[(bt + 1) & 1]);
#pragma unroll
            for (int i = 0; i < RO_KB2; i += 2) {
              if (kb + i < KS) acc0 = __builtin_amdgcn_mfma_f64_16x16x4f64(af[bt & 1][i], act[(kb + i) * AR + bl], acc0, 0, 0, 0);
              if (kb + i + 1 < KS)
                acc1 = __builtin_amdgcn_mfma_f64_16x16x4f64(af[bt & 1][i + 1], act[(kb + i + 1) * AR + bl], acc1, 0, 0, 0);
            }
          }
        }
        if (mine) {
          const int col = lane & 15;
#pragma unroll
          for (int r = 0; r < 4; ++r) {
            const int row = 16 * wv + (lane >> 4) + 4 * r;
            const double v = acc0[r] + acc1[r];
            if (last) sPsi[row * 16 + col] = v;
            else if (NW != 8 || col < 8) actn[(row >> 2) * AR + (row & 3) * (AR / 4) + col] = v > 0.0 ? v : 0.0;
          }
        }
        if (!last) {
          if (h + 1 < R.nhh) { if (hid) ro_load_afrags(R.Whp[h + 1], KS, wv, 0, lane, af[0]); }
          else if (out) ro_load_afrags(R.Wop, KS, wv, 0, lane, af[0]);
        }
        LSTAMP(3 + 2 * h);
        __syncthreads();
        LSTAMP(4 + 2 * h);
      }
      }
      if ((lane & PSI_MASK) < L) psi_i = sPsi[(lane & PSI_MASK) * 16 + wv];
    }

#ifdef KMPC_TRACE
    if (lane == 0 && b < 8192) kmpc_trace_buf[b * 32 + 17] = wall_clock64();
    if (lane == 0 && b < 8192 && k == 0) {
      kmpc_trace_buf[b * 32 + 29] = (unsigned long long)__builtin_amdgcn_s_getreg((3 << 11) | 20) | ((unsigned long long)__builtin_amdgcn_s_getreg((31 << 11) | 4) << 8);
      kmpc_trace_buf[b * 32 + 19] = wall_clock64();
      for (int sl = 22; sl < 29; ++sl) kmpc_trace_buf[b * 32 + sl] = 0ull;
    }
#endif
    if (live) {
      int woff = R.wbase + wv * R.wstride, bk = b;
      asm volatile("" : "+s"(woff), "+s"(bk));
      double* const wsm = smem + woff;
      double* const psi_now = R.psi[cur];
      if (lane < L) psi_now[(size_t)b * L + lane] = psi_i;
      V2DiagOut dgo{nullptr, nullptr, nullptr};
      if constexpr (DIAG) {
        if (R.Psi_log && lane < L) io_st<IOT>(R.Psi_log, ((size_t)k * L + lane) * B + b, psi_i);
        const size_t kb = (size_t)k * B + b;
        dgo.dA = R.dA_log ? io_at<IOT>(R.dA_log, kb) : nullptr;
        dgo.dB = R.dB_log ? io_at<IOT>(R.dB_log, kb) : nullptr;
        dgo.dC = R.dC_log ? io_at<IOT>(R.dC_log, kb) : nullptr;
      }
      StepVar<double> sv;
      sv.psi_now = psi_now;
      sv.psi_prev = R.psi[cur ^ 1];
      sv.psi_in_regs = 1;
      sv.psi_now_v = psi_i;
      sv.psi_prev_v = psi_prev_reg;
      sv.phases = PH_CONDENSE | PH_QP | ((have_prev && !R.no_update) ? PH_RLS : 0);
      sv.first_update = fresh ? 1 : 0;
      sv.plant_switched = (R.switch_step >= 0 && R.step0 + k >= R.switch_step) ? 1 : 0;
      sv.U0 = R.U_log ? io_at<IOT>(R.U_log, (size_t)k * B) : a.U0;
      sv.x_next = RBF ? nullptr : sXn + wv * 4;
      sv.cov_done = (k > 0 && !R.no_update) ? 1 : 0;
      const bool tile_wave = RBF || NW == 4 || wv < ((KS_ > 0 ? (KS_ <= 28 ? 112 : 128) : R.Hp) >> 4) || wv < (R.Lp >> 4);
      sv.cov_ahead = (k + 1 < R.steps && !R.no_update && tile_wave) ? 1 : 0;
      if constexpr (DIAG) {
        if (!(sv.phases & PH_RLS) && lane == 0) {
          if (dgo.dA) io_st<IOT>(dgo.dA, 0, 0.0);
          if (dgo.dB) io_st<IOT>(dgo.dB, 0, 0.0);
          if (dgo.dC) io_st<IOT>(dgo.dC, 0, 0.0);
        }
      }
      constexpr bool LOWREG = ro_max_threads<L_, N_, Q_, NW, KS_>() == 1024 && N_ > 24;
      if constexpr (TERM) {
        StepVar<double> sv1 = sv, sv2 = sv;
        sv1.phases = sv.phases & PH_RLS;
        sv1.cov_ahead = 0;
        sv2.phases = sv.phases & ~PH_RLS;
        double* imgb = V2 ? R.img + (size_t)bk * R.img_stride : nullptr;
        if (sv1.phases) {
          if constexpr (V2) step_v2<L_, N_, Q_, LOWREG, !LOWREG, IOT, 1, DIAG>(a, sv1, bk, wsm, imgb, &dgo);
          else step_body<double, 64, L_, N_, Q_, LOWREG, !LOWREG || Q_ == L_, ro_one_region<L_, N_, Q_, KS_>()>(a, sv1, bk, wsm);
        }
        __threadfence_block();
        block_sync<64>();
        if (R.term_every > 0 && ((R.term_count0 + k) % R.term_every) == 0) {
          double* const scr = R.term_scratch + (size_t)bk * R.term_scratch_stride;
          double* const Wb = R.term_W + (size_t)bk * Q_ * Q_;
          int itd;
          if constexpr (V2) {
            const V2Dims vd(L_, 2);
            const int cy0 = a.cy0;
            itd = wave_dare(L_, Q_, [&](int i, int j) { return imgb[vd.off1(i, j)]; }, [&](int r, int j) { return imgb[vd.off1(L_ + cy0 + r, j)]; },
                            R.term_Q, R.term_R, R.term_eps, R.term_maxiter, a.Qw, scr, Wb);
          } else {
            const double* const Kb = a.K + (size_t)bk * a.strideK;
            const double* const Cb = a.C + (size_t)bk * a.strideC;
            const int cy0 = a.cy0;
            itd = wave_dare(L_, Q_, [&](int i, int j) { return Kb[i * (L_ + 1) + j]; },
                            [&](int r, int j) { return Q_ == L_ ? (r == j ? 1.0 : 0.0) : Cb[(cy0 + r) * L_ + j]; },
                            R.term_Q, R.term_R, R.term_eps, R.term_maxiter, a.Qw, scr, Wb);
          }
          if (R.term_iters && lane == 0) R.term_iters[bk] = itd;
        }
        if constexpr (V2) step_v2<L_, N_, Q_, LOWREG, !LOWREG, IOT, 2>(a, sv2, bk, wsm, imgb);
        else step_body<double, 64, L_, N_, Q_, LOWREG, !LOWREG || Q_ == L_, ro_one_region<L_, N_, Q_, KS_>()>(a, sv2, bk, wsm);
      } else if constexpr (V2) {
        double* imgb = R.img + (size_t)bk * R.img_stride;
        step_v2<L_, N_, Q_, LOWREG, !LOWREG, IOT, 0, DIAG>(a, sv, bk, wsm, imgb, &dgo);
      } else {
        step_body<double, 64, L_, N_, Q_, LOWREG, !LOWREG || Q_ == L_, ro_one_region<L_, N_, Q_, KS_>()>(a, sv, bk, wsm);
      }
      if (R.X_log) {
        __threadfence_block();
        if (lane < n) io_st<IOT>(R.X_log, ((size_t)k * n + lane) * B + b, io_ld<IOT>(a.X_rw, (size_t)lane * B + b));
      }
    }
#ifdef KMPC_TRACE
    if (lane == 0 && b < 8192) {
      const unsigned long long t18 = wall_clock64();
      kmpc_trace_buf[b * 32 + 18] = t18;
      const unsigned long long dl = kmpc_trace_buf[b * 32 + 17] - kmpc_trace_buf[b * 32 + 16], db = t18 - kmpc_trace_buf[b * 32 + 17];
      if (b < 4096 && k < 32) {
        kmpc_step_buf[b * 96 + 3 * k] = (unsigned)kmpc_trace_buf[b * 32 + 16];
        kmpc_step_buf[b * 96 + 3 * k + 1] = (unsigned)kmpc_trace_buf[b * 32 + 17];
        kmpc_step_buf[b * 96 + 3 * k + 2] = (unsigned)t18;
      }
      kmpc_trace_buf[b * 32 + 20] = (k == 0 ? 0ull : kmpc_trace_buf[b * 32 + 20]) + dl;
      kmpc_trace_buf[b * 32 + 21] = (k == 0 ? 0ull : kmpc_trace_buf[b * 32 + 21]) + db;
    }
#endif
    if (have_prev) fresh = false;
    have_prev = true;
    cur ^= 1;
    psi_prev_reg = psi_i;
  }
  if (!RBF && live && (tid0 & 63) == 0) {
    const int* const acc = reinterpret_cast<const int*>(sXn + wave * 4 + 2);
    if (ra.s.status) ra.s.status[b] = acc[0];
    if (ra.s.iters) ra.s.iters[b] = acc[1];
    if (ra.work) ra.work[b] = acc[2];
  }
}


static int ro_one_region_r2(int n, int L, int q, int N) { return n * L <= N * q ? 0 : ((n * L + 1) & ~1); }
static size_t ro_step_lds_elems(int n, int L, int q, int N, int* r1, int* r2, bool lds_tableau) {
  if (r1) *r1 = step_region1(L, N);
  if (r2) *r2 = step_region2(n, L, N, lds_tableau);
  return step_lds_elems(n, L, q, N, lds_tableau);
}
static size_t rollout_lds_elems(int n, int L, int q, int N, bool rbf, int waves, int Lp, int* wstride) {
  size_t per_wave = (ro_step_lds_elems(n, L, q, N, nullptr, nullptr, !tableau_saves_lds(N, L)) + 1) & ~(size_t)1;
  if (ro_one_region_rt(L, N, q, rbf))
    per_wave = ((size_t)step_region1(L, N) + ro_one_region_r2(n, L, q, N) + vec_elems_one_region(n, L, q, N) + 1) & ~(size_t)1;
  const bool v2 = step_v2_dims(L, N, q);
  if (v2) per_wave = v2_lds_elems(L, q, N);
  if (wstride) *wstride = (int)per_wave;
  size_t elems = per_wave * waves;
  if (rbf) return elems;
  const size_t scratch = ro_scratch_of(waves);
  if (v2) return scratch + elems + ro_keep(Lp, waves);
  if (elems < scratch) elems = scratch;
  return elems + ro_keep(Lp, waves);
}
#if defined(KMPC_ROLLOUT_JIT_TU)
static int g_rollout_workgroup = 0;
#elif defined(KMPC_ROLLOUT_IO32_TU)
extern int g_rollout_workgroup;
#else
int g_rollout_workgroup = 0;
void set_rollout_workgroup(int trajectories) { g_rollout_workgroup = trajectories; }
#endif
static int rollout_waves(int n, int L, int q, int N, bool rbf, int Lp, int B = 1 << 30) {
  const size_t cap = 160 * 1024 / sizeof(double);
  if (!rbf) {
    static const char* env = dbg_env("KMPC_ROLLOUT_WAVES");
    auto wgs = [&](int w) -> int {
      const size_t e = (rollout_lds_elems(n, L, q, N, false, w, Lp, nullptr) + 63) & ~(size_t)63;
      const int k = (int)(cap / e);
      const int maxw = (N > 24 && !ro_one_region_rt(L, N, q, false) && !step_v2_dims(L, N, q)) ? 8 : 16;
      return k * w > maxw ? maxw / w : k;
    };
    if (g_rollout_workgroup) return wgs(g_rollout_workgroup) > 0 ? g_rollout_workgroup : 0;
    if (env && (atoi(env) == 4 || atoi(env) == 8 || atoi(env) == 16)) return wgs(atoi(env)) > 0 ? atoi(env) : 0;
    static int cus_dev[16] = {};
    int& cus = cus_dev[device_slot()];
    if (!cus) {
      int dev = 0;
      if (hipGetDevice(&dev) != hipSuccess || hipDeviceGetAttribute(&cus, hipDeviceAttributeMultiprocessorCount, dev) != hipSuccess || cus <= 0) cus = 256;
    }
    int best = 0, best_traj = 0;
    for (int w = 16; w >= 8; w >>= 1) {
      const int t = wgs(w) * w;
      if (t > best_traj) { best = w; best_traj = t; }
    }
    if (wgs(4) * 4 >= 2 * best_traj && wgs(4) > 0) { best = 4; best_traj = wgs(4) * 4; }
    if (best == 16 && wgs(8) * 8 >= 16 && (B + 15) / 16 < cus) return 8;
    return best;
  }
  for (int w = ro_rbf_eight(L, N, q) ? 8 : 16; w >= 4; --w)
    if (rollout_lds_elems(n, L, q, N, true, w, Lp, nullptr) <= cap) return w;
  return 0;
}
template <int L_, int N_, int Q_, int NW, int KS_, typename IOT = double, bool TERM = false, bool DIAG = false>
static hipError_t launch_rollout_nw(const RolloutArgs<double>& k, int waves, size_t lds, hipStream_t s) {
  static size_t configured_dev[16] = {};
  size_t& configured = configured_dev[device_slot()];
  if (lds > 64 * 1024 && lds > configured) {
    hipError_t e = hipFuncSetAttribute(reinterpret_cast<const void*>(&rollout_kernel<L_, N_, Q_, NW, KS_, IOT, TERM, DIAG>),
                                       hipFuncAttributeMaxDynamicSharedMemorySize, (int)lds);
    if (e != hipSuccess) return e;
    configured = lds;
  }
  const int grid = (k.s.B + waves - 1) / waves;
  hipLaunchKernelGGL((rollout_kernel<L_, N_, Q_, NW, KS_, IOT, TERM, DIAG>), dim3(grid), dim3(64 * waves), lds, s, k);
  return hipGetLastError();
}

template <int L_, int N_, int Q_, typename IOT = double> static hipError_t launch_rollout_impl(const RolloutArgs<double>& a, hipStream_t s, int waves_in = 0) {
  RolloutArgs<double> k = a;
  const bool rbf = a.lift_rbf != 0;
  constexpr bool V2 = ro_v2<L_, N_, Q_>();
  int waves = waves_in > 0 ? waves_in : rollout_waves(a.s.n, a.s.L, a.s.q, a.s.N, rbf, a.Lp, a.s.B);
  if (sizeof(IOT) == 4 && !rbf && waves == 4) waves = 8;
  if (waves == 0) return hipErrorInvalidValue;
  ro_step_lds_elems(a.s.n, a.s.L, a.s.q, a.s.N, &k.s.r1, &k.s.r2, !tableau_saves_lds(a.s.N, a.s.L));
  if (!a.s.qp_scratch) return hipErrorInvalidValue;
  if (ro_one_region_rt(a.s.L, a.s.N, a.s.q, rbf)) k.s.r2 = ro_one_region_r2(a.s.n, a.s.L, a.s.q, a.s.N);
  if constexpr (V2) {
    if (!a.img || a.s.n != 2) return hipErrorInvalidValue;
    k.s.r1 = v2_region1(N_);
    k.s.r2 = 0;
  }
  const size_t elems = rollout_lds_elems(a.s.n, a.s.L, a.s.q, a.s.N, rbf, waves, a.Lp, &k.wstride);
  k.keep_off = rbf ? 0 : (int)(elems - ro_keep(a.Lp, waves));
  k.wbase = (V2 && !rbf) ? (int)ro_scratch_of(waves) : 0;
  const size_t lds = elems * sizeof(double);
  if (lds > 160 * 1024) return hipErrorInvalidValue;
  const bool ks25 = !rbf && a.KS == 25 && a.Hp == 112;
#ifdef KMPC_ROLLOUT_JIT_TU
  constexpr int JKS = KMPC_JIT_KS, JNW = JKS < 0 ? 16 : KMPC_JIT_NW;
  if (rbf != (JKS < 0)) return hipErrorInvalidValue;
  if (rbf && (a.rbf_matlab > 1) != (JKS == -2)) return hipErrorInvalidValue;
  if (!rbf && (waves != JNW || ks25 != (JKS == 25))) return hipErrorInvalidValue;
  if ((a.term_every > 0) != (KMPC_JIT_TERM != 0)) return hipErrorInvalidValue;
  if (a.term_every > 0 && (!a.term_Q || !a.term_W || !a.term_scratch || a.term_scratch_stride < term_scratch_elems(L_) || !a.s.Wterm || !a.s.wterm_per_traj))
    return hipErrorInvalidValue;
  if ((a.diag != 0) != (KMPC_JIT_DIAG != 0)) return hipErrorInvalidValue;
  return launch_rollout_nw<L_, N_, Q_, JNW, JKS, IOT, KMPC_JIT_TERM != 0, KMPC_JIT_DIAG != 0>(k, waves, lds, s);
#else
  if (rbf && a.rbf_matlab > 1) return hipErrorInvalidValue;
  if (rbf) return launch_rollout_nw<L_, N_, Q_, 16, -1, IOT>(k, waves, lds, s);
  if constexpr (sizeof(IOT) == 4) {
    if (waves == 16) return ks25 ? launch_rollout_nw<L_, N_, Q_, 16, 25, IOT>(k, waves, lds, s) : launch_rollout_nw<L_, N_, Q_, 16, 0, IOT>(k, waves, lds, s);
    if (waves == 8) return ks25 ? launch_rollout_nw<L_, N_, Q_, 8, 25, IOT>(k, waves, lds, s) : launch_rollout_nw<L_, N_, Q_, 8, 0, IOT>(k, waves, lds, s);
    return hipErrorInvalidValue;
  } else {
  constexpr size_t pw = V2 ? v2_lds_elems(L_, Q_, N_)
                        : ro_one_region<L_, N_, Q_, 0>()
                            ? (((size_t)step_region1(L_, N_) + (2 * L_ <= N_ * Q_ ? 0 : ((2 * L_ + 1) & ~1)) + vec_elems_one_region(2, L_, Q_, N_) + 1) & ~(size_t)1)
                            : ((step_lds_elems(2, L_, Q_, N_, step_tableau_in_lds<64, N_, L_>()) + 1) & ~(size_t)1);
  constexpr size_t cap = 160 * 1024 / sizeof(double);
  if constexpr (4 * pw <= cap)
    if (waves == 4) return ks25 ? launch_rollout_nw<L_, N_, Q_, 4, 25>(k, waves, lds, s) : launch_rollout_nw<L_, N_, Q_, 4, 0>(k, waves, lds, s);
  if constexpr (8 * pw <= cap)
    if (waves == 8) return ks25 ? launch_rollout_nw<L_, N_, Q_, 8, 25>(k, waves, lds, s) : launch_rollout_nw<L_, N_, Q_, 8, 0>(k, waves, lds, s);
  if constexpr (16 * pw <= cap)
    if (waves == 16) return ks25 ? launch_rollout_nw<L_, N_, Q_, 16, 25>(k, waves, lds, s) : launch_rollout_nw<L_, N_, Q_, 16, 0>(k, waves, lds, s);
  return hipErrorInvalidValue;
  }
#endif
}

#ifndef KMPC_DEV_CFG2_ONLY
#define KMPC_FULL_BUILD(...) __VA_ARGS__
#define KMPC_LIFT_BUILD(...) __VA_ARGS__
#else
#define KMPC_FULL_BUILD(...)
#ifdef KMPC_DEV_LIFT
#define KMPC_LIFT_BUILD(...) __VA_ARGS__
#else
#define KMPC_LIFT_BUILD(...)
#endif
#endif
#define KMPC_ROLLOUT_SETS_F64(X)                                                        \
  X(20, 20, 2)  X(8, 30, 2)    \
  KMPC_LIFT_BUILD(X(8, 10, 8) X(8, 30, 8))                                              \
  KMPC_FULL_BUILD(X(8, 10, 2) X(10, 20, 1)  X(20, 30, 2)  X(32, 40, 2)  X(32, 40, 1))
#define KMPC_ROLLOUT_SETS_F32(X) X(20, 20, 2)  KMPC_FULL_BUILD(X(8, 30, 2) X(8, 10, 2) X(10, 20, 1) X(20, 30, 2))
#define KMPC_SET_IS(L_, N_, q_) || (L == L_ && N == N_ && q == q_)
#define KMPC_SET_LAUNCH(L_, N_, q_) if (a.s.L == L_ && a.s.N == N_ && a.s.q == q_) return launch_rollout_impl<L_, N_, q_, IOT>(a, s);
#if defined(KMPC_ROLLOUT_JIT_TU)
#elif defined(KMPC_ROLLOUT_IO32_TU)
hipError_t launch_rollout_io32(const RolloutArgs<double>& a, hipStream_t s) {
  if (a.s.B <= 0 || a.steps <= 0) return hipSuccess;
  if (!a.lift_rbf && (a.Hp > 128 || (a.Hp & 15) || a.Lp > 64 || a.KS > 32 || a.nhh < 0 || a.nhh > 2 || a.s.n > 4))
    return hipErrorInvalidValue;
  using IOT = float;
  KMPC_ROLLOUT_SETS_F32(KMPC_SET_LAUNCH)
  return hipErrorInvalidValue;
}
#else
#ifdef KMPC_TRACE
hipError_t launch_rollout_io32(const RolloutArgs<double>&, hipStream_t) { return hipErrorInvalidValue; }
#else
hipError_t launch_rollout_io32(const RolloutArgs<double>& a, hipStream_t s);
#endif
bool rollout_builtin(int L, int N, int q, bool io32) {
  static const bool force = dbg_env("KMPC_FORCE_PLUGIN") != nullptr;
  if (force) return false;
  return io32 ? (false KMPC_ROLLOUT_SETS_F32(KMPC_SET_IS)) : (false KMPC_ROLLOUT_SETS_F64(KMPC_SET_IS));
}
bool rollout_io32_available(int n, int L, int N, int q, bool rbf) {
#ifdef KMPC_TRACE
  return false;
#endif
  return n == 2 && step_v2_dims(L, N, q) && rollout_fused_available<double>(n, L, N, q, 64, rbf);
}
template <typename T> bool rollout_fused_available(int n, int L, int N, int q, int threads, bool rbf) {
  if (sizeof(T) != 8 || threads == 256 || n > 4) return false;
  const bool inst = rollout_builtin(L, N, q, false) || rollout_plugin_dims(n, L, N, q);
  return inst && rollout_waves(n, L, q, N, rbf, 64) > 0;
}
bool rollout_plugin_key(int n, int L, int N, int q, bool rbf, int Lp, int KS, int Hp, int B, bool io32, RolloutPluginKey* out, bool term, bool diag,
                        bool rbf_kinds) {
  rbf_kinds = rbf_kinds && rbf;
  if ((!term && !diag && !rbf_kinds && rollout_builtin(L, N, q, io32)) || !rollout_plugin_dims(n, L, N, q)) return false;
  if (term && io32) return false;
  if (diag && (io32 || !rollout_uses_image(n, L, N, q))) return false;
  if (io32 && !step_v2_dims(L, N, q)) return false;
  int waves = rollout_waves(n, L, q, N, rbf, Lp, B);
  if (io32 && !rbf && waves == 4) waves = 8;
  if (waves == 0) return false;
  out->L = L; out->N = N; out->q = q; out->io32 = io32 ? 1 : 0; out->term = term ? 1 : 0; out->diag = diag ? 1 : 0;
  out->ks = rbf ? (rbf_kinds ? -2 : -1) : ((KS == 25 && Hp == 112) ? 25 : 0);
  out->nw = rbf ? 16 : waves;
  return true;
}
static hipError_t launch_rollout_plugin(const RolloutArgs<double>& a, const RolloutPlugin* p, hipStream_t s) {
  if (!p || !p->fn) return hipErrorInvalidValue;
  const int waves = p->key.ks < 0 ? rollout_waves(a.s.n, a.s.L, a.s.q, a.s.N, true, a.Lp, a.s.B) : p->key.nw;
  return p->fn(&a, waves, s);
}
bool rollout_uses_image(int n, int L, int N, int q) { return n == 2 && step_v2_dims(L, N, q); }
template <> hipError_t launch_rollout_fused<double>(const RolloutArgs<double>& a, hipStream_t s, const RolloutPlugin* plugin) {
  if (a.s.B <= 0 || a.steps <= 0) return hipSuccess;
  if (!a.lift_rbf && (a.Hp > 128 || (a.Hp & 15) || a.Lp > 64 || a.KS > 32 || a.nhh < 0 || a.nhh > 2 || a.s.n > 4))
    return hipErrorInvalidValue;
  if (a.term_every > 0 || a.diag || (a.lift_rbf && a.rbf_matlab > 1) || !rollout_builtin(a.s.L, a.s.N, a.s.q, a.io_f32 != 0)) return launch_rollout_plugin(a, plugin, s);
  if (a.io_f32) return launch_rollout_io32(a, s);
  using IOT = double;
  KMPC_ROLLOUT_SETS_F64(KMPC_SET_LAUNCH)
  return hipErrorInvalidValue;
}
template <> hipError_t launch_rollout_fused<float>(const RolloutArgs<float>&, hipStream_t, const RolloutPlugin*) { return hipErrorInvalidValue; }
template bool rollout_fused_available<float>(int, int, int, int, int, bool);
template bool rollout_fused_available<double>(int, int, int, int, int, bool);

#endif

}
```

koopman-online-updated-mpc_amd/csrc/step_body.h:

```cpp
#pragma once
#include "kernels.h"
#include "plant_device.h"

#ifdef KMPC_TRACE
__device__ unsigned long long kmpc_trace_buf[8192 * 32];
#define KTRACE(slot)                                                                                      \
  do {                                                                                                    \
    if (tid == 0 && b < 8192) kmpc_trace_buf[b * 32 + (slot)] = wall_clock64();                          \
  } while (0)
extern "C" int kmpc_trace_read(void* host, size_t bytes) {
  return (int)hipMemcpyFromSymbol(host, HIP_SYMBOL(kmpc_trace_buf), bytes, 0, hipMemcpyDeviceToHost);
}
#else
#define KTRACE(slot)
#endif

namespace kmpc {

static constexpr int imax(int a, int b) { return a > b ? a : b; }

static constexpr int vec_elems(int n, int L, int q, int N) {
  const int p = L + 1;
  const int setA = 2 * p + 6 * L + n + 2 * N * q;
  const int setB = 3 * N;
  return imax(setA, setB) + N  + 16 ;
}

static constexpr int vec_elems_one_region(int n, int L, int q, int N) {
  return 5 * L + n + 2 * N * q + N + 16;
}
static constexpr int step_region1(int L, int N) { return (imax(imax((L + 1) * (L + 1), L * L), N * N) + 1) & ~1; }
static constexpr int step_region2(int n, int L, int N, bool lds_tableau = true) {
  return (imax(L * (L + 1) + n * L, lds_tableau ? N * N : 0) + 1) & ~1;
}
static constexpr size_t step_lds_elems(int n, int L, int q, int N, bool lds_tableau = true) {
  return (size_t)step_region1(L, N) + step_region2(n, L, N, lds_tableau) + vec_elems(n, L, q, N);
}

template <int TPB> __device__ __forceinline__ void block_sync() {
  if constexpr (TPB == 64) {
    __builtin_amdgcn_fence(__ATOMIC_RELEASE, "wavefront");
    __builtin_amdgcn_wave_barrier();
    __builtin_amdgcn_fence(__ATOMIC_ACQUIRE, "wavefront");
  } else {
    __syncthreads();
  }
}
template <int TPB> __device__ __forceinline__ void block_sync_lds() {
  if constexpr (TPB == 64) {
    block_sync<TPB>();
  } else {
    asm volatile("s_waitcnt lgkmcnt(0)\n\ts_barrier" ::: "memory");
  }
}
template <int TPB> __device__ __forceinline__ int local_tid() {
  int t = TPB == 64 ? (int)__builtin_amdgcn_mbcnt_hi(~0u, __builtin_amdgcn_mbcnt_lo(~0u, 0u)) : (int)threadIdx.x;
  asm volatile("" : "+v"(t));
  return t;
}

template <typename T> struct StepVar {
  int phases, first_update, plant_switched;
  const T* psi_prev;
  const T* psi_now;
  T* U0;
  T* x_next;
  int psi_in_regs;
  T psi_now_v, psi_prev_v;
  bool h_global = false;
  int cov_done = 0, cov_ahead = 0;
};

template <int TPB, int COUNT, typename F> __device__ __forceinline__ void for_strided(int tid, int count, F&& f) {
  if constexpr (COUNT > 0) {
    constexpr int IT = (COUNT + TPB - 1) / TPB;
#pragma unroll
    for (int i = 0; i < IT; ++i) {
      const int e = tid + i * TPB;
      if ((i + 1) * TPB <= COUNT || e < COUNT) f(e, i);
    }
  } else {
    int i = 0;
    for (int e = tid; e < count; e += TPB, ++i) f(e, i);
  }
}

static constexpr bool tableau_saves_lds(int N, int L) { return N * N > L * (L + 1) + 4 * L; }
template <int TPB, int N_, int L_> constexpr bool step_tableau_in_lds() {
  return !(N_ > 0 && L_ > 0 && ((TPB == 64 && N_ <= 40) || (TPB == 256 && N_ <= 64)) && tableau_saves_lds(N_, L_));
}

template <int TPB, int L_, int N_, int Q_> constexpr bool step_one_region() {
  return TPB == 256 && L_ > 0 && N_ > 0 && Q_ > 0 && Q_ != L_ && Q_ <= 2 && (L_ & 3) == 0 && L_ <= 64 &&
         ((L_ + 1) * (L_ + 1) + TPB - 1) / TPB <= 17;
}

template <typename T> struct Tol;
template <> struct Tol<double> {
  static __device__ __forceinline__ double kkt() { return 1e-9; }
  static __device__ __forceinline__ double tight() { return 1e-12; }
  static __device__ __forceinline__ double act() { return 1e-8; }
  static __device__ __forceinline__ double slack() { return 1e-14; }
};
template <> struct Tol<float> {
  static __device__ __forceinline__ float kkt() { return 2e-5f; }
  static __device__ __forceinline__ float tight() { return 2.4e-7f; }
  static __device__ __forceinline__ float act() { return 1e-5f; }
  static __device__ __forceinline__ float slack() { return 1e-6f; }
};

__device__ __forceinline__ double tfma(double a, double b, double c) { return __builtin_fma(a, b, c); }
__device__ __forceinline__ float tfma(float a, float b, float c) { return __builtin_fmaf(a, b, c); }
__device__ __forceinline__ double tabs(double v) { return __builtin_fabs(v); }
__device__ __forceinline__ float tabs(float v) { return __builtin_fabsf(v); }
typedef __attribute__((address_space(3))) double lds_f64;
typedef __attribute__((address_space(3))) int lds_i32;
typedef __attribute__((address_space(3))) float lds_f32;
__device__ __forceinline__ double lds_ld(const double* p) { return *(const lds_f64*)p; }
__device__ __forceinline__ void lds_st(double* p, double v) { *(lds_f64*)p = v; }
__device__ __forceinline__ float lds_ld(const float* p) { return *(const lds_f32*)p; }
__device__ __forceinline__ void lds_st(float* p, float v) { *(lds_f32*)p = v; }
__device__ __forceinline__ double uniform_value(double v) {
  return __hiloint2double(__builtin_amdgcn_readfirstlane(__double2hiint(v)), __builtin_amdgcn_readfirstlane(__double2loint(v)));
}
__device__ __forceinline__ float uniform_value(float v) { return __int_as_float(__builtin_amdgcn_readfirstlane(__float_as_int(v))); }
template <typename T> __device__ __forceinline__ T tclip(T v, T lo, T hi) { return v < lo ? lo : (v > hi ? hi : v); }
template <typename IOT, typename T> __device__ __forceinline__ T io_ld(const T* base, size_t i) { return (T) reinterpret_cast<const IOT*>(base)[i]; }
template <typename IOT, typename T> __device__ __forceinline__ void io_st(T* base, size_t i, T v) { reinterpret_cast<IOT*>(base)[i] = (IOT)v; }
template <typename IOT, typename T> __device__ __forceinline__ T* io_at(T* base, size_t i) { return reinterpret_cast<T*>(reinterpret_cast<IOT*>(base) + i); }
template <typename IOT, typename T> __device__ __forceinline__ const T* io_at(const T* base, size_t i) { return reinterpret_cast<const T*>(reinterpret_cast<const IOT*>(base) + i); }

template <int LANE, bool NOP>
__device__ __forceinline__ void fmac_rowbcast(double& acc, double vec, double coef) {
  if constexpr (NOP)
    asm volatile("s_nop 1\n\tv_fmac_f64_dpp %0, %1, %2 row_newbcast:%3 row_mask:0xf bank_mask:0xf"
                 : "+v"(acc) : "v"(vec), "v"(coef), "n"(LANE));
  else
    asm volatile("v_fmac_f64_dpp %0, %1, %2 row_newbcast:%3 row_mask:0xf bank_mask:0xf"
                 : "+v"(acc) : "v"(vec), "v"(coef), "n"(LANE));
}
struct RowAsm {
  char s[2048];
  int n;
  constexpr const char* data() const { return s; }
  constexpr size_t size() const { return (size_t)n; }
};
template <int L0, int L1, bool PAD> constexpr RowAsm row_dot_text() {
  RowAsm t{};
  auto put = [&t](const char* p) { while (*p) t.s[t.n++] = *p++; };
  auto num = [&t](int v) { if (v >= 10) t.s[t.n++] = (char)('0' + v / 10); t.s[t.n++] = (char)('0' + v % 10); };
  if (PAD) put("s_nop 1\n\t");
  for (int l = L0; l < L1; ++l) {
    put("v_fmac_f64_dpp %0, %"); num(l < 16 ? 1 : 2); put(", %"); num(3 + l - L0);
// ... 2173 lines not shown
```

koopman-online-updated-mpc_amd/csrc/step_v2.h:

```cpp
#pragma once
#include "step_body.h"
#include <type_traits>
#include "qp_rl.h"

namespace kmpc {

static constexpr bool step_v2_dims(int L, int N, int q) { return q != L && q > 0 && q <= 2 && L + 2 <= 32 && N <= 32 && L >= 2; }
static constexpr int v2_region1(int N) { return (N * rl_stride(N) + 1) & ~1; }
static constexpr int v2_cov_elems(int L) { return 32 + ((L + 1) & ~1); }
static constexpr int v2_carry_elems(int L) { return 66 + v2_cov_elems(L); }
static constexpr bool v2_chain_dump(int N) { return N < 30; }
static constexpr int v2_vec_elems(int q, int N) { return 16 + 2 * ((N + 1) & ~1) + (q + 2 * N * q) + imax(2 * N, (N + 1) * q + (v2_chain_dump(N) ? (N + 1) * q + 64 : 0)) + 2; }
static constexpr size_t v2_lds_elems(int L, int q, int N) { return ((size_t)v2_region1(N) + v2_carry_elems(L) + v2_vec_elems(q, N) + 1) & ~(size_t)1; }

template <int CNT, int NCOL, bool BLK = true>
__device__ __forceinline__ void rowdot_one(double& ac, double v0, double v1, const double (&R)[NCOL]) {
  row_dot<CNT, BLK>(ac, v0, v1, R);
}
template <int CNT, int NCOL, int LOWCOL>
__device__ __forceinline__ void rowupd(double (&R)[NCOL], double v0, double v1, double coef) {
  row_upd<CNT, LOWCOL>(R, v0, v1, coef);
}
template <int B, int E, typename F> __device__ __forceinline__ void static_for(F&& f) {
  if constexpr (B < E) {
    f(std::integral_constant<int, B>{});
    static_for<B + 1, E>(f);
  }
}
template <int CNT, int OFF> __device__ __forceinline__ void lds_store2_lanes(double* p1, double* p2, double v) {
  typedef __attribute__((address_space(3))) double* lds_t;
  const unsigned a1 = (unsigned)(size_t)(lds_t)p1, a2 = (unsigned)(size_t)(lds_t)p2;
  constexpr unsigned LO = CNT >= 32 ? 0xffffffffu : ((1u << CNT) - 1u), HI = CNT > 32 ? ((1u << (CNT - 32)) - 1u) : 0u;
  unsigned long long saved;
  asm volatile("s_mov_b64 %0, exec\n\ts_mov_b32 exec_lo, %4\n\ts_mov_b32 exec_hi, %5\n\tds_write_b64 %1, %3 offset:%6\n\t"
               "ds_write_b64 %2, %3 offset:%6\n\ts_mov_b64 exec, %0"
               : "=&s"(saved) : "v"(a1), "v"(a2), "v"(v), "n"(LO), "n"(HI), "n"(OFF) : "memory");
}
template <int ROWS> __device__ __forceinline__ void gather_rows(double a, double& v0, double& v1) {
  if constexpr (ROWS <= 16) { v0 = a; v1 = a; }
  else half_gather(a, v0, v1);
}
__device__ __forceinline__ void halves_both(double a, double& lo, double& hi) {
  const int al = __double2loint(a), ah = __double2hiint(a);
  const auto rl = __builtin_amdgcn_permlane32_swap(al, al, false, false);
  const auto rh = __builtin_amdgcn_permlane32_swap(ah, ah, false, false);
  lo = __hiloint2double(rh[0], rl[0]);
  hi = __hiloint2double(rh[1], rl[1]);
}

template <int L_, bool SYNC>
__device__ __forceinline__ double v2_rls_cov(double* const img, const double z, const double lam) {
  typedef double d2_t __attribute__((ext_vector_type(2)));
  constexpr int P_ = L_ + 1, CP = (L_ + 2) / 2, NC = 2 * CP, S2 = 2 * L_ + 1;
  const int tid = local_tid<64>(), half = tid >> 5, t = tid & 31;
  const d2_t* const im = reinterpret_cast<const d2_t*>(img);
  d2_t* const imw = reinterpret_cast<d2_t*>(img);
  const int slot2 = half ? P_ + (t < L_ ? t : L_ - 1) : (t < P_ ? t : P_ - 1);
  double R2[NC];
#pragma unroll
  for (int c = 0; c < CP; ++c) {
    const d2_t v = im[c * S2 + slot2];
    R2[2 * c] = v.x; R2[2 * c + 1] = v.y;
  }
  if constexpr (SYNC) __syncthreads();
  double zv0, zv1;
  gather_rows<P_>(z, zv0, zv1);
  double acc2 = 0.0;
  rowdot_one<P_, NC>(acc2, zv0, zv1, R2);
  double s = ((half && t >= L_) ? 0.0 : z) * acc2;
  s += dpp_shr(s, 1);
  s += dpp_shr(s, 2);
  s += dpp_shr(s, 4);
  s += dpp_shr(s, 8);
  double rt = 0.0;
  fmac_rowbcast<15, true>(rt, s, 1.0);
  double r0, r1 = 0.0;
  if constexpr (P_ <= 16) r0 = rt;
  else half_gather(rt, r0, r1);
  const double dd = (half ? 1.0 : lam) + (r0 + r1);
  const double dinv = 1.0 / dd;
  const double c2 = -acc2 * dinv;
  if constexpr (SYNC) __syncthreads();
  double w0, w1;
  gather_rows<P_>(acc2, w0, w1);
  rowupd<P_, NC, L_>(R2, w0, w1, c2);
  if (lam != 1.0) {
    const double sc = half ? 1.0 : 1.0 / lam;
#pragma unroll
    for (int c = 0; c < P_; ++c) R2[c] *= sc;
  }
  if (half ? t < L_ : t < P_) {
#pragma unroll
    for (int c = 0; c < CP; ++c) {
      d2_t v;
      v.x = R2[2 * c]; v.y = R2[2 * c + 1];
      imw[c * S2 + slot2] = v;
    }
  }
  return acc2 * dinv;
}
template <int N_> __device__ __forceinline__ double* v2_cov_slot(double* sm) { return sm + v2_region1(N_) + 66; }
template <int L_> __device__ __forceinline__ int v2_cov_index(int lane) { return lane < 32 ? lane : (lane - 32 < L_ ? lane : 32 + L_ - 1 + (L_ & 1)); }

struct V2DiagOut { double* dA; double* dB; double* dC; };
template <int L_, int N_, int Q_, bool LOWREG, bool ASREG, typename IOT = double, int PART = 0, bool DIAG = false>
__device__ __forceinline__ void step_v2(const StepArgs<double>& a, const StepVar<double>& sv, const int b, double* const sm, double* const img,
                                        const V2DiagOut* const dg = nullptr) {
  typedef double d2_t __attribute__((ext_vector_type(2)));
  constexpr int P_ = L_ + 1, CP = (L_ + 2) / 2, NC = 2 * CP, NX = 2, S2 = 2 * L_ + 1, S1 = L_ + NX;
  constexpr int N = N_, q = Q_;
  static_assert(step_v2_dims(L_, N_, Q_), "step_v2: dimension set");
  static_assert(N_ <= 32 && L_ + 2 <= 32, "step_v2: one variable / one state row per lane of a 32-lane half");
  const int tid = local_tid<64>();
  const int half = tid >> 5, t = tid & 31;
  const int B = a.B;
  double* const sR = sm;
  double* const sCs = sR + v2_region1(N_);
  double* const sCov = sCs + 66;
  double* const vec = sCs + v2_carry_elems(L_);
  double* const red = vec;
  constexpr int NE = (N_ + 1) & ~1;
  double* const sf = red + 16;
  double* const qxo = sf + NE;
  double* const sEr = qxo + NE + q;
  double* const sG = sEr + 2 * N * q;
  double* const dump = sG + (N + 1) * q;
  double* const qxa = sG;
  double* const qg = qxa + N;

  KTRACE(0);
  const double up = uniform_value(a.u_prev[b]);
  double xw_pre = 0.0;
  constexpr int REFN = (Q_ * N_ + 63) / 64;
  double refp[REFN];
  if (sv.phases & PH_CONDENSE) {
    const double* refg = io_at<IOT>(a.ref, a.ref_per_traj ? (size_t)b * q * N : 0);
#pragma unroll
    for (int i = 0; i < REFN; ++i) {
      const int e = tid + i * 64, ec = e < q * N ? e : 0, k = ec / q, r = ec - k * q;
      refp[i] = io_ld<IOT>(refg, r * N + k);
    }
  }

  double R1[NC];
  const int slot1 = t < S1 ? t : S1 - 1;
  const d2_t* const im = reinterpret_cast<const d2_t*>(img);
  d2_t* const imw = reinterpret_cast<d2_t*>(img);
  const double psin = sv.psi_now_v;
  if (PART != 2 && (sv.phases & PH_RLS)) {
    const bool fu = sv.first_update != 0;
    if (!fu) {
#pragma unroll
      for (int c = 0; c < CP; ++c) {
        const d2_t v = im[CP * S2 + c * S1 + slot1];
        R1[2 * c] = v.x; R1[2 * c + 1] = v.y;
      }
    } else {
#pragma unroll
      for (int c = 0; c < NC; ++c) R1[c] = 0.0;
    }
    const int xr = t - L_ < 0 ? 0 : (t - L_ < NX ? t - L_ : NX - 1);
    double xn;
    if (sv.x_next) xn = lds_ld(sv.x_next + xr);
    else xn = io_ld<IOT>(a.x_now, (size_t)xr * B + b);
    const double z = t < L_ ? sv.psi_prev_v : (t == L_ ? up : 0.0);
    KTRACE(1);
    const double u2 = sv.cov_done ? sCov[v2_cov_index<L_>(tid)] : v2_rls_cov<L_, false>(img, z, a.lam);
    KTRACE(2);
    double zv0, zv1;
    gather_rows<(S1 > P_ ? S1 : P_)>(z, zv0, zv1);
    double acc1 = 0.0;
    rowdot_one<P_, NC>(acc1, zv0, zv1, R1);
    KTRACE(3);
    {
      double gall, hall;
      halves_both(u2, gall, hall);
      double g0, g1, h0, h1;
      gather_rows<(S1 > P_ ? S1 : P_)>(gall, g0, g1);
      gather_rows<(S1 > P_ ? S1 : P_)>(hall, h0, h1);
      const bool isK = t < L_, isC = t >= L_ && t < S1;
      double eK = psin - acc1;
      if (a.lam != 1.0) {
        const double linv = 1.0 / a.lam;
        eK = eK * linv + psin * (1.0 - linv);
        const double sc = isK ? linv : 1.0;
#pragma unroll
        for (int c = 0; c < P_; ++c) R1[c] *= sc;
      }
      const double cK = isK ? eK : 0.0;
      const double cC = (isC && !(a.c_skip_first && fu)) ? xn - acc1 : 0.0;
      rowupd<P_, NC, -1>(R1, g0, g1, cK);
      rowupd<L_, NC, -1>(R1, h0, h1, cC);
      if constexpr (DIAG) {
        double s1 = half ? cC * cC : cK * cK;
        double s2 = t < L_ ? (half ? hall * hall : gall * gall) : 0.0;
        s1 += dpp_shr(s1, 1); s2 += dpp_shr(s2, 1);
        s1 += dpp_shr(s1, 2); s2 += dpp_shr(s2, 2);
        s1 += dpp_shr(s1, 4); s2 += dpp_shr(s2, 4);
        s1 += dpp_shr(s1, 8); s2 += dpp_shr(s2, 8);
        const double e2 = lane_bcast(s1, 15) + lane_bcast(s1, 31), ec2 = lane_bcast(s1, 47) + lane_bcast(s1, 63);
        const double g2 = lane_bcast(s2, 15) + lane_bcast(s2, 31), h2 = lane_bcast(s2, 47) + lane_bcast(s2, 63);
        const double gL = lane_bcast(gall, L_);
        const double en = __builtin_sqrt(e2), qn = __builtin_nan("");
        if (tid == 0) {
          if (dg->dA) io_st<IOT>(dg->dA, 0, fu ? qn : en * __builtin_sqrt(g2));
          if (dg->dB) io_st<IOT>(dg->dB, 0, fu ? qn : en * __builtin_fabs(gL));
          if (dg->dC) io_st<IOT>(dg->dC, 0, fu ? qn : __builtin_sqrt(ec2) * __builtin_sqrt(h2));
        }
      }
      if (!half && t < S1) {
#pragma unroll
        for (int c = 0; c < CP; ++c) {
          d2_t v;
          v.x = R1[2 * c]; v.y = R1[2 * c + 1];
          imw[CP * S2 + c * S1 + slot1] = v;
        }
      }
    }
    KTRACE(4);
  } else if (PART != 1) {
#pragma unroll
    for (int c = 0; c < CP; ++c) {
      const d2_t v = im[CP * S2 + c * S1 + slot1];
      R1[2 * c] = v.x; R1[2 * c + 1] = v.y;
    }
  }
  if constexpr (PART == 1) return;

  {
    const bool isA = t < L_;
    double v0, v1;
    gather_rows<S1>(isA ? (half ? psin : R1[L_]) : 0.0, v0, v1);
    const double bs = (a.du_mode && isA) ? R1[L_] * (half ? up : 1.0) : 0.0;
    const int ro = t - L_ - a.cy0;
    const bool isO = ro >= 0 && ro < q;
    double* const optr = isO ? (half ? sEr - q + ro : sG + ro) : dump + tid;
    KTRACE(5);
    constexpr int JN = N_;
#pragma unroll
    for (int j = 0; j <= JN; ++j) {
      double acc = bs;
      rowdot_one<L_, NC>(acc, v0, v1, R1);
      if constexpr (v2_chain_dump(N_)) optr[j * q] = acc;
      else if (isO) optr[j * q] = acc;
      if (j < JN) gather_rows<S1>(acc, v0, v1);
    }
    block_sync<64>();
#pragma unroll
    for (int i = 0; i < REFN; ++i) {
      const int e = tid + i * 64;
      if (e < q * N) sEr[e] -= refp[i];
    }
    block_sync<64>();
  }
  KTRACE(6);
  if ((sv.phases & PH_QP) && a.x_warm) xw_pre = a.x_warm[(size_t)(t < N_ ? t : 0) * a.B + b];
  double M[N_];
  double rs = 1.0, rsi = 1.0;
  QpCarry cs;
  {
    const int* const ci = reinterpret_cast<const int*>(sCs + 64);
    cs.smask = (unsigned)__builtin_amdgcn_readfirstlane(ci[0]);
    cs.valid = __builtin_amdgcn_readfirstlane(ci[1]);
    cs.umask = (unsigned)__builtin_amdgcn_readfirstlane(ci[2]);
    cs.trust = __builtin_amdgcn_readfirstlane(ci[3]);
    if (cs.valid) {
      const double* const trow = sR + (t < N_ ? t : N_ - 1) * rl_stride(N_);
      if constexpr ((N_ & 1) == 0) {
        const d2_t* t2 = reinterpret_cast<const d2_t*>(__builtin_assume_aligned(trow, 16));
#pragma unroll
        for (int j = 0; j < N_ / 2; ++j) { const d2_t v = t2[j]; M[2 * j] = v.x; M[2 * j + 1] = v.y; }
      } else {
#pragma unroll
        for (int j = 0; j < N_; ++j) M[j] = trow[j];
      }
      rs = sCs[t];
      rsi = sCs[32 + t];
    }
    block_sync<64>();
  }
  {
    typedef double dq_t __attribute__((ext_vector_type(Q_ == 2 ? 2 : 1)));
    const int hf = tid >> 5, idx = tid & 31;
    const dq_t* const gq = reinterpret_cast<const dq_t*>(__builtin_assume_aligned(sG, Q_ == 2 ? 16 : 8));
    const dq_t* const wq = reinterpret_cast<const dq_t*>(__builtin_assume_aligned((hf ? sEr : sG) + idx * Q_, Q_ == 2 ? 16 : 8));
    double acc = 0.0;
    constexpr int NS = rl_stride(N_);
    double* const h1 = sR - idx * NS;
    double* const h2 = sR - idx;
    const double Qw = a.Qw, rdiag = idx == 0 ? a.Rw : 0.0;
    constexpr int HCH = 10;
    static_for<0, (N_ + HCH - 1) / HCH>([&](auto CC) {
      constexpr int c0 = decltype(CC)::value * HCH, c1 = c0 + HCH < N_ ? c0 + HCH : N_;
      double hv[HCH];
      static_for<c0, c1>([&](auto TT) {
        constexpr int tt = decltype(TT)::value;
        if constexpr (Q_ == 2) {
          const dq_t u = gq[tt], w = wq[tt];
          acc = tfma(u[0], w[0], acc);
          acc = tfma(u[1], w[1], acc);
        } else {
#pragma unroll
          for (int r = 0; r < Q_; ++r) acc = tfma(sG[tt * Q_ + r], ((hf ? sEr : sG) + idx * Q_)[tt * Q_ + r], acc);
        }
        hv[tt - c0] = Qw * acc + rdiag;
      });
      static_for<c0, c1>([&](auto TT) {
        constexpr int tt = decltype(TT)::value;
        lds_store2_lanes<N_ - tt, (N_ - 1 - tt) * (NS + 1) * 8>(h1, h2, hv[tt - c0]);
      });
    });
    if (hf && idx < N_) sf[idx] = 2.0 * Qw * acc;
  }
  if (a.Wterm) {
    block_sync<64>();
    const double* const Wt = a.Wterm + (a.wterm_per_traj ? (size_t)b * q * q : (size_t)0);
    for (int e = tid; e < N * N; e += 64) {
      const int aa = e / N, bb = e - aa * N;
      const double* ga = sG + (N - 1 - aa) * q;
      const double* gb = sG + (N - 1 - bb) * q;
      double acc = 0.0;
#pragma unroll 1
      for (int r = 0; r < q; ++r)
#pragma unroll 2
        for (int s2 = 0; s2 < q; ++s2) acc += ga[r] * (0.5 * (Wt[r * q + s2] + Wt[s2 * q + r])) * gb[s2];
      sR[aa * rl_stride(N_) + bb] += acc;
    }
    for (int aa = tid; aa < N; aa += 64) {
      const double* ga = sG + (N - 1 - aa) * q;
      const double* eN = sEr + (N - 1) * q;
      double acc = 0.0;
#pragma unroll 1
      for (int r = 0; r < q; ++r)
#pragma unroll 2
        for (int s2 = 0; s2 < q; ++s2) acc += ga[r] * Wt[r * q + s2] * eN[s2];
      sf[aa] += 2.0 * acc;
    }
  }
  block_sync<64>();
  KTRACE(7);

  if (sv.phases & PH_QP) {
    if (qp_rl<N_, IOT>(sR, sf, a, sv, b, qxo, red + 15, M, rs, rsi, cs, up, xw_pre)) {
#ifdef KMPC_TRACE
      if (tid == 0 && b < 8192) kmpc_trace_buf[b * 32 + 28] += 1ull;
#endif
      block_sync<64>();
      double* const Hg = a.qp_scratch + (size_t)b * N * N;
      for (int e = tid; e < N * N; e += 64) Hg[e] = sR[(e / N) * rl_stride(N_) + (e % N)];
      __threadfence_block();
      block_sync<64>();
      qp_lds<double, 64, IOT>(Hg, sf, sR, qxo, qxa, qg, red, a, sv, b, N, true);
      block_sync<64>();
      for (int e = tid; e < N * q; e += 64) sEr[N * q + e] = 0.0;
      if (tid == 0) red[15] = qxo[0];
    }
    if (!half) {
      sCs[t] = rs;
      sCs[32 + t] = rsi;
    }
    if (tid == 0) {
      int* const ci = reinterpret_cast<int*>(sCs + 64);
      ci[0] = (int)cs.smask;
      ci[1] = cs.valid;
      ci[2] = (int)cs.umask;
      ci[3] = cs.trust;
    }
    block_sync<64>();
    if (sv.cov_ahead) {
      const double uk = (a.du_mode ? up : 0.0) + red[15];
      const double gains = v2_rls_cov<L_, false>(img, t < L_ ? psin : (t == L_ ? uk : 0.0), a.lam);
      if (!half || t < L_) sCov[v2_cov_index<L_>(tid)] = gains;
    }
  }
}

template <int L_, int N_, int Q_> __device__ __forceinline__ void step_v2_init(double* const sm) {
  const int tid = local_tid<64>();
  double* const sCs = sm + v2_region1(N_);
  double* const sEr = sCs + v2_carry_elems(L_) + 16 + 2 * ((N_ + 1) & ~1) + Q_;
  if (tid == 0) {
    int* const ci = reinterpret_cast<int*>(sCs + 64);
    ci[0] = 0;
    ci[1] = 0;
    ci[2] = 0;
    ci[3] = 0;
  }
  for (int e = tid; e < N_ * Q_; e += 64) sEr[N_ * Q_ + e] = 0.0;
}

}
```

koopman-online-updated-mpc_amd/koopmpc/_ffi.py:

```python
from __future__ import annotations

import ctypes as C
import os

_PKG_DIR = os.path.dirname(os.path.abspath(__file__))
LIB_PATH = os.environ.get("KMPC_LIB") or os.path.join(os.path.dirname(_PKG_DIR), "libkoopmpc.so")

KMPC_F32, KMPC_F64 = 0, 1
KMPC_LIFT_MLP, KMPC_LIFT_RBF_PY, KMPC_LIFT_RBF_MATLAB = 0, 1, 2
KMPC_LIFT_RBF_GAUSS, KMPC_LIFT_RBF_INVQUAD, KMPC_LIFT_RBF_INVMULTQUAD, KMPC_LIFT_RBF_POLYHARMONIC = 3, 4, 5, 6
KMPC_OUT_CX, KMPC_OUT_LIFT = 0, 1
KMPC_PLANT_DUFFING, KMPC_PLANT_VDP, KMPC_PLANT_TANK = 0, 1, 2
KMPC_PLANT_RK4_MATLAB = 16
KMPC_LIFT_OFFSET_NONE, KMPC_LIFT_OFFSET_PSI0, KMPC_LIFT_OFFSET_X_PSI0 = 0, 1, 2


class KmpcConfig(C.Structure):
    _fields_ = [
        ("n", C.c_int32), ("m", C.c_int32), ("L", C.c_int32), ("N", C.c_int32),
        ("hidden", C.c_int32), ("layers", C.c_int32), ("lift_kind", C.c_int32),
        ("output_kind", C.c_int32), ("dtype", C.c_int32), ("batch", C.c_int32),
        ("qp_max_iter", C.c_int32), ("threads", C.c_int32),
        ("delta_u", C.c_int32), ("out_row0", C.c_int32), ("out_rows", C.c_int32), ("c_skip_first", C.c_int32),
        ("cold_start", C.c_int32), ("lift_offset", C.c_int32),
        ("lam", C.c_double), ("P0", C.c_double), ("barQ0", C.c_double),
        ("Qw", C.c_double), ("Rw", C.c_double), ("lb", C.c_double), ("ub", C.c_double),
        ("rbf_eps", C.c_double), ("umin", C.c_double), ("umax", C.c_double),
    ]


_VP, _I, _I64, _D = C.c_void_p, C.c_int, C.c_int64, C.c_double
_DP = C.POINTER(C.c_double)
SIGNATURES = {
    "kmpc_create": (_I, [C.POINTER(KmpcConfig), C.POINTER(_VP)]),
    "kmpc_destroy": (_I, [_VP]),
    "kmpc_last_error": (C.c_char_p, [_VP]),
    "kmpc_version": (_I, []),
    "kmpc_set_encoder": (_I, [_VP, _I, _DP, _DP, _I, _I]),
    "kmpc_set_encoder_layer": (_I, [_VP, _I, _DP, _DP, _I, _I]),
    "kmpc_set_centres": (_I, [_VP, _DP, _I, _I]),
    "kmpc_set_rbf_order": (_I, [_VP, _I]),
    "kmpc_set_model": (_I, [_VP, _DP, _DP, _DP]),
    "kmpc_set_terminal_weight": (_I, [_VP, _DP]),
    "kmpc_solve_dare": (_I, [_VP, _VP, _DP, _D, _I, _D, _I, _I, _VP, _VP, _VP, _VP]),
    "kmpc_terminal_from_dare": (_I, [_VP, _DP, _D, _I, _D, _I, _DP, C.POINTER(C.c_int32), _VP]),
    "kmpc_set_terminal_refresh": (_I, [_VP, _I, _DP, _D, _I, _D]),
    "kmpc_rollout_is_fused": (_I, [_VP]),
    "kmpc_rollout_plugin_status": (_I, [_VP, C.c_char_p, _I]),
    "kmpc_rollout_plugin_prebuild": (_I, [_I, _I, _I, _I, _I, _I, _I, _I, C.c_char_p, _I]),
    "kmpc_set_rollout_workgroup": (_I, [_I]),
    "kmpc_rank_by_work": (_I, [_VP, _I, _VP, _VP]),
    "kmpc_reset": (_I, [_VP, _VP]),
    "kmpc_state_init": (_I, [_VP, _D, _D, _VP]),
    "kmpc_state_init_from": (_I, [_VP, _DP, _DP, _DP, _DP, _VP]),
    "kmpc_lift": (_I, [_VP, _VP, _VP, _I, _VP]),
    "kmpc_rls_update": (_I, [_VP, _VP, _VP, _VP, _VP, _I, _VP]),
    "kmpc_get_model": (_I, [_VP, _VP, _VP, _VP, _VP]),
    "kmpc_condense": (_I, [_VP, _VP, _VP, _I, _VP, _VP, _I, _VP]),
    "kmpc_condense_cost": (_I, [_VP, _VP, _VP, _I, _VP, _VP, _VP, _I, _VP]),
    "kmpc_mpc_solve": (_I, [_VP, _VP, _VP, _VP, _I, _VP, _VP, _I, _D, _D, _D, _D, _DP, _VP, _VP, _VP, _VP, _VP, _I, _VP]),
    "kmpc_qp_solve": (_I, [_VP, _VP, _VP, _VP, _VP, _VP, _I, _VP]),
    "kmpc_step": (_I, [_VP, _VP, _VP, _I, _VP, _VP, _VP, _VP, _VP]),
    "kmpc_offline_fit": (_I, [_VP, _VP, _VP, _VP, _I, _D, _I, _VP, _VP, _VP, _VP]),
    "kmpc_generate_and_fit": (_I, [_VP, _I, _VP, _VP, _I, _I, _D, _D, _I, _VP, _VP, _VP, _VP, _VP, _VP]),
    "kmpc_gram_elems": (_I64, [_VP]),
    "kmpc_allreduce_gram": (_I, [_VP, _VP, _VP, _VP]),
    "kmpc_shared_local_gram": (_I, [_VP, _VP, _VP, _VP]),
    "kmpc_gram_accumulate": (_I, [_VP, _VP, _VP, _VP]),
    "kmpc_shared_solve": (_I, [_VP, _VP, _VP, _VP, _VP, _VP, _VP, _VP]),
    "kmpc_shared_solve_plant": (_I, [_VP, _VP, _VP, _VP, _VP, _VP, _VP, _I, _VP, _I, _D, _VP]),
    "kmpc_shared_rollout": (_I, [_VP, _I, _VP, _VP, _I, _I, _I, _D, _VP, _VP, _VP, _VP, _VP, _VP, _VP, _VP]),
    "kmpc_shared_get_model": (_I, [_VP, _VP, _VP, _VP, _VP]),
    "kmpc_set_applied_input": (_I, [_VP, _VP, _I, _VP]),
    "kmpc_set_online_update": (_I, [_VP, _I]),
    "kmpc_plant_step": (_I, [_VP, _I, _VP, _VP, _D, _I, _I, _VP]),
    "kmpc_rollout": (_I, [_VP, _I, _VP, _VP, _I, _I, _I, _I, _D, _VP, _VP, _VP, _VP, _VP]),
    "kmpc_set_rollout_diagnostics": (_I, [_VP, _I]),
    "kmpc_estimator_status": (_I, [_VP, _DP, _DP]),
    "kmpc_get_prev_transition": (_I, [_VP, _VP, _VP, _VP]),
    "kmpc_rollout_diag": (_I, [_VP, _I, _VP, _VP, _I, _I, _I, _I, _D, _VP, _VP, _VP, _VP, _VP, _VP, _VP, _VP, _VP]),
    "kmpc_rollout_diag_plugin_prebuild": (_I, [_I, _I, _I, _I, _I, _I, _I, _I, C.c_char_p, _I]),
    "kmpc_state_bytes": (_I64, [_VP]),
    "kmpc_state_export": (_I, [_VP, _VP, _I64]),
    "kmpc_state_import": (_I, [_VP, _VP, _I64]),
    "kmpc_profile_enable": (_I, [_VP, _I]),
    "kmpc_profile_read": (_I, [_VP, _DP, C.POINTER(_I64), _I]),
    "kmpc_algorithmic_bytes_per_step": (_I64, [_VP]),
}

_lib = None


def load():
    global _lib
    if _lib is not None:
        return _lib
    import torch

    if not os.path.exists(LIB_PATH):
        raise ImportError(
            "koopmpc: %s is missing. Build the HIP library first (python __graft_entry__.py, or "
            "make -C koopman-online-updated-mpc_amd); koopmpc has no CPU path." % LIB_PATH
        )
    lib = C.CDLL(LIB_PATH)
    for name, (res, args) in SIGNATURES.items():
        fn = getattr(lib, name)
        fn.restype = res
        fn.argtypes = args
    _lib = lib
    return lib


class KmpcError(RuntimeError):
    pass


def check(lib, handle, rc, what):
    if rc != 0:
        msg = lib.kmpc_last_error(handle)
        raise KmpcError("%s failed (%d): %s" % (what, rc, (msg or b"").decode("utf-8", "replace")))
```

koopman-online-updated-mpc_amd/koopmpc/api.py:

```python
from __future__ import annotations

import ctypes as C

import numpy as np
import torch

from . import _ffi
from .sharding import force_collectives


def _dptr(a):
    return np.ascontiguousarray(a, dtype=np.float64).ctypes.data_as(C.POINTER(C.c_double))


def solve_DARE(A, B, Q, R, maxiter=500, eps=0.01, device="cuda:0", return_iters=False):
    P, K, it = _dare(A, B, Q, R, maxiter, eps, device, want_gain=False)
    return (P, it) if return_iters else P


def dlqr(A, B, Q, R, maxiter=500, eps=0.01, device="cuda:0"):
    P, K, it = _dare(A, B, Q, R, maxiter, eps, device, want_gain=True)
    return K


# ... 408 lines not shown
        self._chk(self.lib.kmpc_rollout_diag(self.h, plant, self._p(X), self._p(rr), per, int(steps), int(step0), int(switch_step), float(h),
                                             self._p(Ul), self._p(Xl), self._p(Psi), self._p(dA), self._p(dB), self._p(dC),
                                             self._p(st), self._p(it), self._stream()), "kmpc_rollout_diag")

    def estimator_status(self):
        P0, Q0 = C.c_double(), C.c_double()
        bits = int(self.lib.kmpc_estimator_status(self.h, C.byref(P0), C.byref(Q0)))
        if bits < 0:
            self._chk(bits, "kmpc_estimator_status")
        return bool(bits & 1), bool(bits & 2), P0.value, Q0.value

    def rollout_diagnostics(self, kind, X, r, steps, step0=0, switch_step=102, h=0.05):
        if getattr(self, "_diag_route", None) is None:
            self.set_rollout_diagnostics(True)
        plant = self._plant_id(kind)
        assert X.is_cuda and X.dtype == self.dtype and X.is_contiguous() and tuple(X.shape) == (self.n, self.B)
        rr, per = self._ref(r)
        steps = int(steps)
        kw = dict(dtype=self.dtype, device=self.device)
        Ul, Xl = torch.empty(steps, self.B, **kw), torch.empty(steps, self.n, self.B, **kw)
        Psi = torch.empty(steps, self.L, self.B, **kw)
        dA, dB, dC = (torch.empty(steps, self.B, **kw) for _ in range(3))
        have_prev, pending, P0, Q0 = self.estimator_status()
        kf = (0 if have_prev else 1) if pending else steps
        if kf < steps:
            A0, B0, C0 = self.get_model()
            if have_prev:
                psi_p, u_p, x_k = torch.empty(self.B, self.L, **kw), torch.empty(self.B, **kw), X.clone()
                self._chk(self.lib.kmpc_get_prev_transition(self.h, self._p(psi_p), self._p(u_p), self._stream()), "kmpc_get_prev_transition")
        self._rollout_diag_raw(plant, X, rr, per, steps, step0, switch_step, h, Ul, Xl, Psi, dA, dB, dC, self.status, self.iters)
        if kf < steps:
            if not have_prev:
                psi_p, u_p, x_k = Psi[0].t(), Ul[0], Xl[0]
            psi_k = Psi[kf].t()
            z = torch.cat([psi_p, u_p.reshape(self.B, 1)], dim=1)
            g = P0 * z / (1.0 + P0 * (z * z).sum(dim=1, keepdim=True))
            K1 = psi_k.unsqueeze(2) * g.unsqueeze(1)
            dA[kf] = torch.linalg.matrix_norm(K1[:, :, :self.L] - A0, ord=2)
            dB[kf] = torch.linalg.vector_norm(K1[:, :, self.L] - B0.reshape(self.B, self.L), dim=1)
            if C0 is not None:
                hv = Q0 * psi_p / (1.0 + Q0 * (psi_p * psi_p).sum(dim=1, keepdim=True))
                C1 = x_k.t().unsqueeze(2) * hv.unsqueeze(1)
                if self.cfg.c_skip_first:
                    C1 = torch.zeros_like(C1)
                dC[kf] = torch.linalg.matrix_norm(C1 - C0, ord=2)
            else:
                dC[kf] = 0.0
        self._keep = (rr,)
        return Ul, Xl, {"Psi": Psi, "dA": dA, "dB": dB, "dC": dC}

    def state_dict(self):
        nb = self.lib.kmpc_state_bytes(self.h)
        buf = np.empty(nb, dtype=np.uint8)
        self._chk(self.lib.kmpc_state_export(self.h, C.c_void_p(buf.ctypes.data), nb), "kmpc_state_export")
        return {"blob": buf}

    def state_to(self, blob=None):
        nb = self.lib.kmpc_state_bytes(self.h)
        if blob is None:
            blob = torch.empty(nb, dtype=torch.uint8, device=self.device)
        assert blob.dtype == torch.uint8 and blob.numel() >= nb and blob.is_contiguous()
        self._chk(self.lib.kmpc_state_export(self.h, C.c_void_p(blob.data_ptr()), nb), "kmpc_state_export")
        return blob

    def state_from(self, blob):
        self._chk(self.lib.kmpc_state_import(self.h, C.c_void_p(blob.data_ptr()), blob.numel()), "kmpc_state_import")

    def load_state_dict(self, sd):
        buf = np.ascontiguousarray(sd["blob"], dtype=np.uint8)
        self._chk(self.lib.kmpc_state_import(self.h, C.c_void_p(buf.ctypes.data), buf.size), "kmpc_state_import")

    def profile(self, on=True):
        self._chk(self.lib.kmpc_profile_enable(self.h, int(on)), "kmpc_profile_enable")

    def profile_read(self, reset=True):
        ms = (C.c_double * 2)()
        cnt = C.c_int64()
        self._chk(self.lib.kmpc_profile_read(self.h, ms, C.byref(cnt), int(reset)), "kmpc_profile_read")
        return {"lift_ms": ms[0], "step_ms": ms[1], "count": cnt.value}

    def rollout_is_fused(self):
        return bool(self.lib.kmpc_rollout_is_fused(self.h))

    def rollout_plugin_status(self):
        buf = C.create_string_buffer(1024)
        code = int(self.lib.kmpc_rollout_plugin_status(self.h, buf, len(buf)))
        return code, buf.value.decode("utf-8", "replace")

    def algorithmic_bytes_per_step(self):
        return int(self.lib.kmpc_algorithmic_bytes_per_step(self.h))


_handles = {}


def _handle(key, make):
    h = _handles.get(key)
    if h is None:
        h = _handles[key] = make()
    return h


class AutoEncoder:

    def __init__(self, weights, device=None, lift_offset=None):
        self.weights = [(np.asarray(W, dtype=np.float64), np.asarray(b, dtype=np.float64).reshape(-1)) for W, b in weights]
        n, L = self.weights[0][0].shape[1], self.weights[-1][0].shape[0]
        if lift_offset == "x_psi0":
            L += n
        self._mpc = KoopmanMPC(n=n, L=L, N=2, batch=1, weights=self.weights, hidden=self.weights[0][0].shape[0],
                               layers=len(self.weights) - 1, device=device, lift_offset=lift_offset)

    def Encoder(self, x):
        return self._mpc.Encoder(x)

    __call__ = Encoder


_RBF_TYPES = {"thinplate": "rbf_matlab", "gauss": "rbf_gauss", "invquad": "rbf_invquad", "invmultquad": "rbf_invmultquad",
              "polyharmonic": "rbf_polyharmonic"}


def _rbf_arguments(eps, form, type, k):
    if type is None:
        return ("rbf" if form == "python" else "rbf_matlab"), (1e-4 if eps is None else float(eps)), 1
    lift = _RBF_TYPES.get(str(type).lower())
    if lift is None:
        raise ValueError("RBF type not recognize")
    if lift != "rbf_polyharmonic":
        k = 1
    elif int(k) != k or not 1 <= int(k) <= 8:
        raise ValueError("the polyharmonic coefficient k must be an integer in 1..8")
    return lift, (1.0 if eps is None else float(eps)), int(k)


def rbf(X, cx, eps=None, form="python", device=None, type=None, k=1):
    lift, eps, k = _rbf_arguments(eps, form, type, k)
    cx = np.ascontiguousarray(cx, dtype=np.float64)
    L, n = cx.shape
    m = _handle(("rbf", L, n, lift, eps, k, str(device)),
                lambda: KoopmanMPC(n=n, L=L, N=2, batch=1, lift=lift, centres=cx, rbf_eps=eps, rbf_k=k, device=device))
    return m.rbf(X, cx)


def costFunction(uSequence, r, AB, C, x0, pastu=None, Np=None, Nc=None, d=None, ek=None, Qw=100.0, Rw=1e-4, device=None):
    U = np.asarray(uSequence.detach().cpu() if torch.is_tensor(uSequence) else uSequence, dtype=np.float64)
    single = U.ndim == 1
    U = U.reshape(U.shape[0], -1)
    N, S = U.shape
    if (Np is not None and Np != N) or (Nc is not None and Nc != N):
        raise ValueError("costFunction: Np = Nc = len(uSequence) is the only setting the reference uses (duffing.py:632-633)")
    if d is not None and np.any(np.asarray(d) != 0.0):
        raise ValueError("costFunction: the offset d is zeros in the reference (duffing.py:776); a non-zero d is not supported")
    AB = np.asarray(AB, dtype=np.float64)
    L = AB.shape[0]
    out = "lift" if C is None else "Cx"
    q = L if C is None else np.asarray(C).shape[0]
    m = _handle(("cost", L, N, S, out, q, float(Qw), float(Rw), str(device)),
                lambda: KoopmanMPC(n=q if C is not None else 2, L=L, N=N, batch=S, lift="rbf", centres=np.zeros((L, q if C is not None else 2)),
                                   output=out, Qw=Qw, Rw=Rw, device=device))
    m.set_model(AB[:, :L], AB[:, L], np.asarray(C, dtype=np.float64) if C is not None else None)
    psi = np.tile(np.asarray(x0, dtype=np.float64).reshape(L, 1), (1, S))
    H, f, c = m.condense(psi, np.asarray(r, dtype=np.float64).reshape(q, N), return_const=True)
    Ud = torch.as_tensor(U.T.copy(), device=m.device)
    J = torch.einsum("si,sij,sj->s", Ud, H, Ud) + (f * Ud).sum(1) + c
    return float(J[0]) if single else J.cpu().numpy()
# ... 29 lines not shown
```

Measured before the change: 152.6 million.

## Add compile-time specialised roll-out kernel for default MPC options

Adds an OPT template parameter and RoOpt traits so that, when runtime options match the defaults (lam=1, no du_mode, warm start, prediction on, fixed max_iter, no logs), the fused roll-out kernel is instantiated with those branches resolved at compile time. The previous applied input is also carried in registers across steps instead of being reloaded from global memory. The aim is to cut kernarg loads, branches and register pressure in the hot loop. In exchange it adds another kernel instantiation plus a variant query API, and the host-side predicate must stay in sync with the compile-time assumptions.

Measured after the change: 156.8 million (median of 6 runs). 2.7% higher.

```diff
diff --git a/include/koopmpc.h b/include/koopmpc.h
--- a/include/koopmpc.h
+++ b/include/koopmpc.h
@@ -142,6 +142,7 @@
 int kmpc_profile_enable(kmpc_handle* h, int on);
 int kmpc_profile_read(kmpc_handle* h, double* ms2, int64_t* count, int reset);
 int kmpc_rollout_is_fused(const kmpc_handle* h);
+int kmpc_rollout_variant(const kmpc_handle* h);
 int kmpc_rollout_plugin_status(const kmpc_handle* h, char* text, int text_bytes);
 int kmpc_rollout_plugin_prebuild(int n, int L, int N, int out_rows, int lift_kind, int hidden_eff, int batch, int dtype, char* text,
                                  int text_bytes);
diff --git a/koopman-online-updated-mpc_amd/csrc/api.hip b/koopman-online-updated-mpc_amd/csrc/api.hip
--- a/koopman-online-updated-mpc_amd/csrc/api.hip
+++ b/koopman-online-updated-mpc_amd/csrc/api.hip
@@ -30,6 +30,7 @@
                                  int32_t* iters_out, hipStream_t s) = 0;
   virtual int set_terminal_refresh(int every, const double* Qh, double R, int maxiter, double eps) = 0;
   virtual int rollout_is_fused() const = 0;
+  int last_rollout_variant = 0;
   virtual int rollout_plugin_status(std::string* text) const = 0;
   virtual int reset(hipStream_t s) = 0;
   virtual int state_init(double P0, double barQ0, hipStream_t s) = 0;
@@ -1193,8 +1194,12 @@
       if (st) HIPCHK(hipMemsetAsync(st, 0, sizeof(int32_t) * (size_t)B, s));
       if (it) HIPCHK(hipMemsetAsync(it, 0, sizeof(int32_t) * (size_t)B, s));
     }
-    if (steps > 0 && fused)
-      return rollout_fused(ctx, plant, X, ref, rpt, steps, step0, switch_step, hs, Ulog, Xlog, st, it, s);
+    if (steps > 0 && fused) {
+      const int rcf = rollout_fused(ctx, plant, X, ref, rpt, steps, step0, switch_step, hs, Ulog, Xlog, st, it, s);
+      if (!rcf) last_rollout_variant = rollout_last_variant();
+      return rcf;
+    }
+    if (steps > 0) last_rollout_variant = 0;
     if (steps == 0 && fused) {
       if constexpr (sizeof(T) == 8) {
         if (use_img) return ensure_image(s);
@@ -1712,6 +1717,7 @@
 }
 int kmpc_set_terminal_refresh(kmpc_handle* h, int every, const double* Q, double R, int maxiter, double eps) { NN(h); return h->set_terminal_refresh(every, Q, R, maxiter, eps); }
 int kmpc_rollout_is_fused(const kmpc_handle* h) { NN(h); return h->rollout_is_fused(); }
+int kmpc_rollout_variant(const kmpc_handle* h) { NN(h); return h->last_rollout_variant; }
 static void put_text(char* text, int text_bytes, const std::string& t) { if (text && text_bytes > 0) snprintf(text, (size_t)text_bytes, "%s", t.c_str()); }
 static int prebuild_variant(int n, int L, int N, int q, bool rbf, int hidden_eff, int batch, bool io32, bool term, bool diag, std::string* text, bool rbf_kinds) {
   const EncoderShape e = encoder_shape(hidden_eff, 0, n, L);
diff --git a/koopman-online-updated-mpc_amd/csrc/kernels.h b/koopman-online-updated-mpc_amd/csrc/kernels.h
--- a/koopman-online-updated-mpc_amd/csrc/kernels.h
+++ b/koopman-online-updated-mpc_amd/csrc/kernels.h
@@ -146,6 +146,7 @@
 std::string rollout_plugin_describe(const RolloutPluginKey& k);
 struct RolloutPlugin { RolloutPluginKey key{}; rollout_plugin_fn fn = nullptr; };
 template <typename T> hipError_t launch_rollout_fused(const RolloutArgs<T>& a, hipStream_t s, const RolloutPlugin* plugin);
+int rollout_last_variant();
 bool rollout_builtin(int L, int N, int q, bool io32);
 bool rollout_plugin_key(int n, int L, int N, int q, bool rbf, int Lp, int KS, int Hp, int B, bool io32, RolloutPluginKey* out, bool term = false,
                         bool diag = false, bool rbf_kinds = false);
diff --git a/koopman-online-updated-mpc_amd/csrc/qp_rl.h b/koopman-online-updated-mpc_amd/csrc/qp_rl.h
--- a/koopman-online-updated-mpc_amd/csrc/qp_rl.h
+++ b/koopman-online-updated-mpc_amd/csrc/qp_rl.h
@@ -106,26 +106,27 @@
   int trust;
 };
 
-template <int N_, typename IOT = double>
+template <int N_, typename IOT = double, int OPT = RO_OPT_GENERIC>
 __device__ __forceinline__ bool qp_rl(double* const sR, const double* sf, const StepArgs<double>& a, const StepVar<double>& sv, const int b,
                                       double* qx_out, double* u_slot, double (&M)[N_], double& rs, double& rsi, QpCarry& cs, double up, double xw_pre) {
   typedef double d2_t __attribute__((ext_vector_type(2)));
+  typedef RoOpt<OPT> O;
   static_assert(N_ <= 32, "qp_rl: one variable per lane of a 32-lane half (ownmask, row_newbcast index, diagonal lane)");
   const int tid = local_tid<64>(), half = tid >> 5, t = tid & 31;
   const bool own = t < N_;
   const int B = a.B;
-  const double uprev = a.du_mode ? up : 0.0;
+  const double uprev = O::du_mode(a) ? up : 0.0;
   double lb = a.lb, ub = a.ub;
   const double tol = Tol<double>::kkt();
   const double eact = Tol<double>::act() * (ub - lb);
   const double xmaxb = tabs(lb) > tabs(ub) ? tabs(lb) : tabs(ub);
-  if (a.du_mode && t == 0) {
+  if (O::du_mode(a) && t == 0) {
     lb = (a.umin - uprev) > lb ? (a.umin - uprev) : lb;
     ub = (a.umax - uprev) < ub ? (a.umax - uprev) : ub;
   }
   const double c0 = tclip(0.0, lb, ub);
-  const bool warm = a.x_warm != nullptr, predict_on = (a.qp_predict & 1) != 0;
-  const int max_iter = a.max_iter;
+  const bool warm = O::warm(a), predict_on = O::predict(a);
+  const int max_iter = O::max_iter(a, N_);
   constexpr unsigned ownmask = N_ >= 32 ? 0xffffffffu : ((1u << N_) - 1u);
   const int rowi = own ? t : N_ - 1;
   constexpr int NS = rl_stride(N_);
@@ -371,15 +372,15 @@
     return true;
   }
   if (own && !half) {
-    if (a.Useq) io_st<IOT>(a.Useq, (size_t)t * B + b, x);
-    if (a.x_warm) a.x_warm[(size_t)t * B + b] = x;
+    if (O::has_useq(a)) io_st<IOT>(a.Useq, (size_t)t * B + b, x);
+    if (O::warm(a)) a.x_warm[(size_t)t * B + b] = x;
   }
   if (tid == 0) {
-    const double uout = a.du_mode ? uprev + x : x;
+    const double uout = O::du_mode(a) ? uprev + x : x;
     *u_slot = x;
-    if (sv.U0) io_st<IOT>(sv.U0, b, uout);
-    if (a.u_store) a.u_store[b] = uout;
-    if (a.plant >= 0) {
+    if (O::has_u0(sv)) io_st<IOT>(sv.U0, b, uout);
+    if (O::has_u_store(a)) a.u_store[b] = uout;
+    if (O::has_plant(a)) {
       double x1, x2;
       if (sv.x_next) { x1 = lds_ld(sv.x_next); x2 = lds_ld(sv.x_next + 1); }
       else { x1 = io_ld<IOT>(a.X_rw, b); x2 = io_ld<IOT>(a.X_rw, (size_t)B + b); }
diff --git a/koopman-online-updated-mpc_amd/csrc/rollout_kernel.hip b/koopman-online-updated-mpc_amd/csrc/rollout_kernel.hip
--- a/koopman-online-updated-mpc_amd/csrc/rollout_kernel.hip
+++ b/koopman-online-updated-mpc_amd/csrc/rollout_kernel.hip
@@ -152,8 +152,11 @@
     LSTAMP(4 + 2 * h);
   }
 }
-template <int L_, int N_, int Q_, int NW, int KS_, typename IOT = double, bool TERM = false, bool DIAG = false>
+template <int L_, int N_, int Q_, int NW, int KS_, typename IOT = double, bool TERM = false, bool DIAG = false, int OPT = RO_OPT_GENERIC>
 __global__ __launch_bounds__((ro_max_threads<L_, N_, Q_, NW, KS_>())) void rollout_kernel(const RolloutArgs<double> ra) {
+  typedef RoOpt<OPT> O;
+#define RO_NO_UPDATE (O::D ? 0 : R.no_update)
+  static_assert(!O::D || (ro_v2<L_, N_, Q_>() && sizeof(IOT) == 8 && !TERM && !DIAG && (KS_ < 0 || NW == 16)), "default-option roll-out: float64 register-state sets");
   static_assert(sizeof(IOT) == 8 || ro_v2<L_, N_, Q_>(), "float32 I/O: register-state dimension sets only");
   static_assert(!DIAG || (sizeof(IOT) == 8 && ro_v2<L_, N_, Q_>()), "diagnostics: float64 register-state dimension sets only");
   extern __shared__ __attribute__((aligned(16))) unsigned char smem_raw[];
@@ -205,10 +208,16 @@
   double psi_prev_reg = 0.0;
   if (live && ra.have_prev && (int)(tid0 & PSI_MASK) < L) psi_prev_reg = ra.psi[ra.cur ^ 1][(size_t)b * L + (tid0 & PSI_MASK)];
   typedef const RolloutArgs<double> __attribute__((address_space(4))) * kernarg_ptr_t;
+  int h_wbase = ra.wbase, h_wstride = ra.wstride;
+  double u_carry = 0.0;
+  (void)u_carry; (void)h_wbase; (void)h_wstride;
   for (int k = 0; k < ra.steps; ++k) {
     kernarg_ptr_t kp = (kernarg_ptr_t)__builtin_amdgcn_kernarg_segment_ptr();
     asm volatile("" : "+s"(kp));
     const RolloutArgs<double> __attribute__((address_space(4)))& R = *kp;
+    if constexpr (O::D) {
+      asm volatile("" : "+s"(h_wbase), "+s"(h_wstride));
+    }
     const StepArgs<double>& a = *(const StepArgs<double>*)(&kp->s);
     int wv = wave;
     asm volatile("" : "+s"(wv));
@@ -323,14 +332,16 @@
       if (V2 && !hid && !out) {
         __syncthreads();
         if constexpr (V2) {
-          if (live && k > 0 && !R.no_update) {
-            int woff0 = R.wbase + wv * R.wstride, bk0 = b;
+          if (live && k > 0 && !RO_NO_UPDATE) {
+            int woff0 = (O::D ? h_wbase : R.wbase) + wv * (O::D ? h_wstride : R.wstride), bk0 = b;
             asm volatile("" : "+s"(woff0), "+s"(bk0));
             double* const wsm0 = smem + woff0;
-            const double uk = a.u_prev[bk0];
+            double uk;
+            if constexpr (O::D) uk = u_carry;
+            else uk = a.u_prev[bk0];
             const int t0 = lane & 31;
             const double z0 = t0 < L_ ? psi_prev_reg : (t0 == L_ ? uk : 0.0);
-            const double gains0 = v2_rls_cov<L_, true>(R.img + (size_t)bk0 * R.img_stride, z0, a.lam);
+            const double gains0 = v2_rls_cov<L_, true>(R.img + (size_t)bk0 * R.img_stride, z0, O::lam(a));
             if (lane < 32 || t0 < L_) v2_cov_slot<N_>(wsm0)[v2_cov_index<L_>(lane)] = gains0;
           } else {
             __syncthreads();
@@ -422,7 +433,7 @@
     }
 #endif
     if (live) {
-      int woff = R.wbase + wv * R.wstride, bk = b;
+      int woff = (O::D ? h_wbase : R.wbase) + wv * (O::D ? h_wstride : R.wstride), bk = b;
       asm volatile("" : "+s"(woff), "+s"(bk));
       double* const wsm = smem + woff;
       double* const psi_now = R.psi[cur];
@@ -441,14 +452,16 @@
       sv.psi_in_regs = 1;
       sv.psi_now_v = psi_i;
       sv.psi_prev_v = psi_prev_reg;
-      sv.phases = PH_CONDENSE | PH_QP | ((have_prev && !R.no_update) ? PH_RLS : 0);
+      sv.phases = PH_CONDENSE | PH_QP | ((have_prev && !RO_NO_UPDATE) ? PH_RLS : 0);
       sv.first_update = fresh ? 1 : 0;
       sv.plant_switched = (R.switch_step >= 0 && R.step0 + k >= R.switch_step) ? 1 : 0;
-      sv.U0 = R.U_log ? io_at<IOT>(R.U_log, (size_t)k * B) : a.U0;
+      if constexpr (O::D) sv.U0 = a.U0;
+      else sv.U0 = R.U_log ? io_at<IOT>(R.U_log, (size_t)k * B) : a.U0;
+      if constexpr (O::D) { sv.u_prev_in_regs = k > 0 ? 1 : 0; sv.u_prev_v = u_carry; }
       sv.x_next = RBF ? nullptr : sXn + wv * 4;
-      sv.cov_done = (k > 0 && !R.no_update) ? 1 : 0;
+      sv.cov_done = (k > 0 && !RO_NO_UPDATE) ? 1 : 0;
       const bool tile_wave = RBF || NW == 4 || wv < ((KS_ > 0 ? (KS_ <= 28 ? 112 : 128) : R.Hp) >> 4) || wv < (R.Lp >> 4);
-      sv.cov_ahead = (k + 1 < R.steps && !R.no_update && tile_wave) ? 1 : 0;
+      sv.cov_ahead = (k + 1 < R.steps && !RO_NO_UPDATE && tile_wave) ? 1 : 0;
       if constexpr (DIAG) {
         if (!(sv.phases & PH_RLS) && lane == 0) {
           if (dgo.dA) io_st<IOT>(dgo.dA, 0, 0.0);
@@ -492,11 +505,12 @@
         else step_body<double, 64, L_, N_, Q_, LOWREG, !LOWREG || Q_ == L_, ro_one_region<L_, N_, Q_, KS_>()>(a, sv2, bk, wsm);
       } else if constexpr (V2) {
         double* imgb = R.img + (size_t)bk * R.img_stride;
-        step_v2<L_, N_, Q_, LOWREG, !LOWREG, IOT, 0, DIAG>(a, sv, bk, wsm, imgb, &dgo);
+        step_v2<L_, N_, Q_, LOWREG, !LOWREG, IOT, 0, DIAG, OPT>(a, sv, bk, wsm, imgb, &dgo);
+        if constexpr (O::D) u_carry = uniform_value(lds_ld(v2_u_slot<L_, N_>(wsm)));
       } else {
         step_body<double, 64, L_, N_, Q_, LOWREG, !LOWREG || Q_ == L_, ro_one_region<L_, N_, Q_, KS_>()>(a, sv, bk, wsm);
       }
-      if (R.X_log) {
+      if (!O::D && R.X_log) {
         __threadfence_block();
         if (lane < n) io_st<IOT>(R.X_log, ((size_t)k * n + lane) * B + b, io_ld<IOT>(a.X_rw, (size_t)lane * B + b));
       }
@@ -529,6 +543,7 @@
 }
 
 
+#undef RO_NO_UPDATE
 static int ro_one_region_r2(int n, int L, int q, int N) { return n * L <= N * q ? 0 : ((n * L + 1) & ~1); }
 static size_t ro_step_lds_elems(int n, int L, int q, int N, int* r1, int* r2, bool lds_tableau) {
   if (r1) *r1 = step_region1(L, N);
@@ -588,21 +603,39 @@
     if (rollout_lds_elems(n, L, q, N, true, w, Lp, nullptr) <= cap) return w;
   return 0;
 }
-template <int L_, int N_, int Q_, int NW, int KS_, typename IOT = double, bool TERM = false, bool DIAG = false>
+template <int L_, int N_, int Q_, int NW, int KS_, typename IOT = double, bool TERM = false, bool DIAG = false, int OPT = RO_OPT_GENERIC>
 static hipError_t launch_rollout_nw(const RolloutArgs<double>& k, int waves, size_t lds, hipStream_t s) {
   static size_t configured_dev[16] = {};
   size_t& configured = configured_dev[device_slot()];
   if (lds > 64 * 1024 && lds > configured) {
-    hipError_t e = hipFuncSetAttribute(reinterpret_cast<const void*>(&rollout_kernel<L_, N_, Q_, NW, KS_, IOT, TERM, DIAG>),
+    hipError_t e = hipFuncSetAttribute(reinterpret_cast<const void*>(&rollout_kernel<L_, N_, Q_, NW, KS_, IOT, TERM, DIAG, OPT>),
                                        hipFuncAttributeMaxDynamicSharedMemorySize, (int)lds);
     if (e != hipSuccess) return e;
     configured = lds;
   }
   const int grid = (k.s.B + waves - 1) / waves;
-  hipLaunchKernelGGL((rollout_kernel<L_, N_, Q_, NW, KS_, IOT, TERM, DIAG>), dim3(grid), dim3(64 * waves), lds, s, k);
+  hipLaunchKernelGGL((rollout_kernel<L_, N_, Q_, NW, KS_, IOT, TERM, DIAG, OPT>), dim3(grid), dim3(64 * waves), lds, s, k);
   return hipGetLastError();
 }
 
+static bool rollout_default_options(const RolloutArgs<double>& a) {
+  const StepArgs<double>& s = a.s;
+  return s.lam == 1.0 && s.du_mode == 0 && s.cy0 == 0 && s.c_skip_first == 0 && s.ref_per_traj == 0 && s.Wterm == nullptr && s.wterm_per_traj == 0 &&
+         s.x_warm != nullptr && (s.qp_predict & 1) == 1 && s.max_iter == 8 * s.N + 40 && s.Useq == nullptr && s.U0 != nullptr && s.u_store != nullptr &&
+         s.u_prev == s.u_store && s.plant >= 0 && s.n == 2 && a.no_update == 0 && a.U_log == nullptr && a.X_log == nullptr && a.io_f32 == 0 &&
+         a.term_every == 0 && a.diag == 0;
+}
+static thread_local int g_rollout_last_variant = 0;
+#if !defined(KMPC_ROLLOUT_JIT_TU) && !defined(KMPC_ROLLOUT_IO32_TU)
+int rollout_last_variant() { return g_rollout_last_variant; }
+#endif
+template <int L_, int N_, int Q_> constexpr bool ro_default_built() {
+#ifdef KMPC_ROLLOUT_JIT_TU
+  return false;
+#else
+  return Q_ == 2 && ((L_ == 20 && N_ == 20) || (L_ == 8 && N_ == 30));
+#endif
+}
 template <int L_, int N_, int Q_, typename IOT = double> static hipError_t launch_rollout_impl(const RolloutArgs<double>& a, hipStream_t s, int waves_in = 0) {
   RolloutArgs<double> k = a;
   const bool rbf = a.lift_rbf != 0;
@@ -636,6 +669,15 @@
   return launch_rollout_nw<L_, N_, Q_, JNW, JKS, IOT, KMPC_JIT_TERM != 0, KMPC_JIT_DIAG != 0>(k, waves, lds, s);
 #else
   if (rbf && a.rbf_matlab > 1) return hipErrorInvalidValue;
+  g_rollout_last_variant = 1;
+  if constexpr (sizeof(IOT) == 8 && ro_default_built<L_, N_, Q_>()) {
+    static const bool generic = dbg_env("KMPC_ROLLOUT_GENERIC") != nullptr;
+    if (!generic && rollout_default_options(a) && (L_ == 20 ? (!rbf && waves == 16 && ks25) : rbf)) {
+      g_rollout_last_variant = 2;
+      if constexpr (L_ == 20) return launch_rollout_nw<L_, N_, Q_, 16, 25, IOT, false, false, RO_OPT_DEFAULT>(k, waves, lds, s);
+      else return launch_rollout_nw<L_, N_, Q_, 16, -1, IOT, false, false, RO_OPT_DEFAULT>(k, waves, lds, s);
+    }
+  }
   if (rbf) return launch_rollout_nw<L_, N_, Q_, 16, -1, IOT>(k, waves, lds, s);
   if constexpr (sizeof(IOT) == 4) {
     if (waves == 16) return ks25 ? launch_rollout_nw<L_, N_, Q_, 16, 25, IOT>(k, waves, lds, s) : launch_rollout_nw<L_, N_, Q_, 16, 0, IOT>(k, waves, lds, s);
@@ -725,6 +767,7 @@
 }
 static hipError_t launch_rollout_plugin(const RolloutArgs<double>& a, const RolloutPlugin* p, hipStream_t s) {
   if (!p || !p->fn) return hipErrorInvalidValue;
+  g_rollout_last_variant = 1;
   const int waves = p->key.ks < 0 ? rollout_waves(a.s.n, a.s.L, a.s.q, a.s.N, true, a.Lp, a.s.B) : p->key.nw;
   return p->fn(&a, waves, s);
 }
@@ -734,7 +777,7 @@
   if (!a.lift_rbf && (a.Hp > 128 || (a.Hp & 15) || a.Lp > 64 || a.KS > 32 || a.nhh < 0 || a.nhh > 2 || a.s.n > 4))
     return hipErrorInvalidValue;
   if (a.term_every > 0 || a.diag || (a.lift_rbf && a.rbf_matlab > 1) || !rollout_builtin(a.s.L, a.s.N, a.s.q, a.io_f32 != 0)) return launch_rollout_plugin(a, plugin, s);
-  if (a.io_f32) return launch_rollout_io32(a, s);
+  if (a.io_f32) { g_rollout_last_variant = 1; return launch_rollout_io32(a, s); }
   using IOT = double;
   KMPC_ROLLOUT_SETS_F64(KMPC_SET_LAUNCH)
   return hipErrorInvalidValue;
diff --git a/koopman-online-updated-mpc_amd/csrc/step_body.h b/koopman-online-updated-mpc_amd/csrc/step_body.h
--- a/koopman-online-updated-mpc_amd/csrc/step_body.h
+++ b/koopman-online-updated-mpc_amd/csrc/step_body.h
@@ -69,6 +69,27 @@
   T psi_now_v, psi_prev_v;
   bool h_global = false;
   int cov_done = 0, cov_ahead = 0;
+  int u_prev_in_regs = 0;
+  T u_prev_v = T(0);
+};
+
+enum { RO_OPT_GENERIC = 0, RO_OPT_DEFAULT = 1 };
+template <int OPT> struct RoOpt {
+  static constexpr bool D = OPT == RO_OPT_DEFAULT;
+  typedef StepArgs<double> A;
+  static __device__ __forceinline__ double lam(const A& a) { if constexpr (D) return 1.0; else return a.lam; }
+  static __device__ __forceinline__ int du_mode(const A& a) { if constexpr (D) return 0; else return a.du_mode; }
+  static __device__ __forceinline__ int cy0(const A& a) { if constexpr (D) return 0; else return a.cy0; }
+  static __device__ __forceinline__ int c_skip_first(const A& a) { if constexpr (D) return 0; else return a.c_skip_first; }
+  static __device__ __forceinline__ int ref_per_traj(const A& a) { if constexpr (D) return 0; else return a.ref_per_traj; }
+  static __device__ __forceinline__ bool has_wterm(const A& a) { if constexpr (D) return false; else return a.Wterm != nullptr; }
+  static __device__ __forceinline__ bool warm(const A& a) { if constexpr (D) return true; else return a.x_warm != nullptr; }
+  static __device__ __forceinline__ bool predict(const A& a) { if constexpr (D) return true; else return (a.qp_predict & 1) != 0; }
+  static __device__ __forceinline__ int max_iter(const A& a, int N) { if constexpr (D) return 8 * N + 40; else return a.max_iter; }
+  static __device__ __forceinline__ bool has_useq(const A& a) { if constexpr (D) return false; else return a.Useq != nullptr; }
+  static __device__ __forceinline__ bool has_u_store(const A& a) { if constexpr (D) return true; else return a.u_store != nullptr; }
+  static __device__ __forceinline__ bool has_plant(const A& a) { if constexpr (D) return true; else return a.plant >= 0; }
+  template <typename SV> static __device__ __forceinline__ bool has_u0(const SV& sv) { if constexpr (D) return true; else return sv.U0 != nullptr; }
 };
 
 template <int TPB, int COUNT, typename F> __device__ __forceinline__ void for_strided(int tid, int count, F&& f) {
diff --git a/koopman-online-updated-mpc_amd/csrc/step_v2.h b/koopman-online-updated-mpc_amd/csrc/step_v2.h
--- a/koopman-online-updated-mpc_amd/csrc/step_v2.h
+++ b/koopman-online-updated-mpc_amd/csrc/step_v2.h
@@ -100,13 +100,15 @@
   return acc2 * dinv;
 }
 template <int N_> __device__ __forceinline__ double* v2_cov_slot(double* sm) { return sm + v2_region1(N_) + 66; }
+template <int L_, int N_> __device__ __forceinline__ double* v2_u_slot(double* sm) { return sm + v2_region1(N_) + v2_carry_elems(L_) + 15; }
 template <int L_> __device__ __forceinline__ int v2_cov_index(int lane) { return lane < 32 ? lane : (lane - 32 < L_ ? lane : 32 + L_ - 1 + (L_ & 1)); }
 
 struct V2DiagOut { double* dA; double* dB; double* dC; };
-template <int L_, int N_, int Q_, bool LOWREG, bool ASREG, typename IOT = double, int PART = 0, bool DIAG = false>
+template <int L_, int N_, int Q_, bool LOWREG, bool ASREG, typename IOT = double, int PART = 0, bool DIAG = false, int OPT = RO_OPT_GENERIC>
 __device__ __forceinline__ void step_v2(const StepArgs<double>& a, const StepVar<double>& sv, const int b, double* const sm, double* const img,
                                         const V2DiagOut* const dg = nullptr) {
   typedef double d2_t __attribute__((ext_vector_type(2)));
+  typedef RoOpt<OPT> O;
   constexpr int P_ = L_ + 1, CP = (L_ + 2) / 2, NC = 2 * CP, NX = 2, S2 = 2 * L_ + 1, S1 = L_ + NX;
   constexpr int N = N_, q = Q_;
   static_assert(step_v2_dims(L_, N_, Q_), "step_v2: dimension set");
@@ -129,12 +131,14 @@
   double* const qg = qxa + N;
 
   KTRACE(0);
-  const double up = uniform_value(a.u_prev[b]);
+  double up;
+  if (O::D && sv.u_prev_in_regs) up = sv.u_prev_v;
+  else up = uniform_value(a.u_prev[b]);
   double xw_pre = 0.0;
   constexpr int REFN = (Q_ * N_ + 63) / 64;
   double refp[REFN];
   if (sv.phases & PH_CONDENSE) {
-    const double* refg = io_at<IOT>(a.ref, a.ref_per_traj ? (size_t)b * q * N : 0);
+    const double* refg = io_at<IOT>(a.ref, O::ref_per_traj(a) ? (size_t)b * q * N : 0);
 #pragma unroll
     for (int i = 0; i < REFN; ++i) {
       const int e = tid + i * 64, ec = e < q * N ? e : 0, k = ec / q, r = ec - k * q;
@@ -165,7 +169,7 @@
     else xn = io_ld<IOT>(a.x_now, (size_t)xr * B + b);
     const double z = t < L_ ? sv.psi_prev_v : (t == L_ ? up : 0.0);
     KTRACE(1);
-    const double u2 = sv.cov_done ? sCov[v2_cov_index<L_>(tid)] : v2_rls_cov<L_, false>(img, z, a.lam);
+    const double u2 = sv.cov_done ? sCov[v2_cov_index<L_>(tid)] : v2_rls_cov<L_, false>(img, z, O::lam(a));
     KTRACE(2);
     double zv0, zv1;
     gather_rows<(S1 > P_ ? S1 : P_)>(z, zv0, zv1);
@@ -180,15 +184,15 @@
       gather_rows<(S1 > P_ ? S1 : P_)>(hall, h0, h1);
       const bool isK = t < L_, isC = t >= L_ && t < S1;
       double eK = psin - acc1;
-      if (a.lam != 1.0) {
-        const double linv = 1.0 / a.lam;
+      if (O::lam(a) != 1.0) {
+        const double linv = 1.0 / O::lam(a);
         eK = eK * linv + psin * (1.0 - linv);
         const double sc = isK ? linv : 1.0;
 #pragma unroll
         for (int c = 0; c < P_; ++c) R1[c] *= sc;
       }
       const double cK = isK ? eK : 0.0;
-      const double cC = (isC && !(a.c_skip_first && fu)) ? xn - acc1 : 0.0;
+      const double cC = (isC && !(O::c_skip_first(a) && fu)) ? xn - acc1 : 0.0;
       rowupd<P_, NC, -1>(R1, g0, g1, cK);
       rowupd<L_, NC, -1>(R1, h0, h1, cC);
       if constexpr (DIAG) {
@@ -231,8 +235,8 @@
     const bool isA = t < L_;
     double v0, v1;
     gather_rows<S1>(isA ? (half ? psin : R1[L_]) : 0.0, v0, v1);
-    const double bs = (a.du_mode && isA) ? R1[L_] * (half ? up : 1.0) : 0.0;
-    const int ro = t - L_ - a.cy0;
+    const double bs = (O::du_mode(a) && isA) ? R1[L_] * (half ? up : 1.0) : 0.0;
+    const int ro = t - L_ - O::cy0(a);
     const bool isO = ro >= 0 && ro < q;
     double* const optr = isO ? (half ? sEr - q + ro : sG + ro) : dump + tid;
     KTRACE(5);
@@ -254,7 +258,7 @@
     block_sync<64>();
   }
   KTRACE(6);
-  if ((sv.phases & PH_QP) && a.x_warm) xw_pre = a.x_warm[(size_t)(t < N_ ? t : 0) * a.B + b];
+  if ((sv.phases & PH_QP) && O::warm(a)) xw_pre = a.x_warm[(size_t)(t < N_ ? t : 0) * a.B + b];
   double M[N_];
   double rs = 1.0, rsi = 1.0;
   QpCarry cs;
@@ -312,7 +316,7 @@
     });
     if (hf && idx < N_) sf[idx] = 2.0 * Qw * acc;
   }
-  if (a.Wterm) {
+  if (O::has_wterm(a)) {
     block_sync<64>();
     const double* const Wt = a.Wterm + (a.wterm_per_traj ? (size_t)b * q * q : (size_t)0);
     for (int e = tid; e < N * N; e += 64) {
@@ -341,7 +345,7 @@
   KTRACE(7);
 
   if (sv.phases & PH_QP) {
-    if (qp_rl<N_, IOT>(sR, sf, a, sv, b, qxo, red + 15, M, rs, rsi, cs, up, xw_pre)) {
+    if (qp_rl<N_, IOT, OPT>(sR, sf, a, sv, b, qxo, red + 15, M, rs, rsi, cs, up, xw_pre)) {
 #ifdef KMPC_TRACE
       if (tid == 0 && b < 8192) kmpc_trace_buf[b * 32 + 28] += 1ull;
 #endif
@@ -368,8 +372,8 @@
     }
     block_sync<64>();
     if (sv.cov_ahead) {
-      const double uk = (a.du_mode ? up : 0.0) + red[15];
-      const double gains = v2_rls_cov<L_, false>(img, t < L_ ? psin : (t == L_ ? uk : 0.0), a.lam);
+      const double uk = (O::du_mode(a) ? up : 0.0) + red[15];
+      const double gains = v2_rls_cov<L_, false>(img, t < L_ ? psin : (t == L_ ? uk : 0.0), O::lam(a));
       if (!half || t < L_) sCov[v2_cov_index<L_>(tid)] = gains;
     }
   }
diff --git a/koopman-online-updated-mpc_amd/koopmpc/_ffi.py b/koopman-online-updated-mpc_amd/koopmpc/_ffi.py
--- a/koopman-online-updated-mpc_amd/koopmpc/_ffi.py
+++ b/koopman-online-updated-mpc_amd/koopmpc/_ffi.py
@@ -46,6 +46,7 @@
     "kmpc_terminal_from_dare": (_I, [_VP, _DP, _D, _I, _D, _I, _DP, C.POINTER(C.c_int32), _VP]),
     "kmpc_set_terminal_refresh": (_I, [_VP, _I, _DP, _D, _I, _D]),
     "kmpc_rollout_is_fused": (_I, [_VP]),
+    "kmpc_rollout_variant": (_I, [_VP]),
     "kmpc_rollout_plugin_status": (_I, [_VP, C.c_char_p, _I]),
     "kmpc_rollout_plugin_prebuild": (_I, [_I, _I, _I, _I, _I, _I, _I, _I, C.c_char_p, _I]),
     "kmpc_set_rollout_workgroup": (_I, [_I]),
diff --git a/koopman-online-updated-mpc_amd/koopmpc/api.py b/koopman-online-updated-mpc_amd/koopmpc/api.py
--- a/koopman-online-updated-mpc_amd/koopmpc/api.py
+++ b/koopman-online-updated-mpc_amd/koopmpc/api.py
@@ -514,6 +514,9 @@
     def rollout_is_fused(self):
         return bool(self.lib.kmpc_rollout_is_fused(self.h))
 
+    def rollout_variant(self):
+        return int(self.lib.kmpc_rollout_variant(self.h))
+
     def rollout_plugin_status(self):
         buf = C.create_string_buffer(1024)
         code = int(self.lib.kmpc_rollout_plugin_status(self.h, buf, len(buf)))
```
